# OpenwaterHealth/OpenLIFU-python

Measured on AMD Instinct MI355X. Metric: Mvoxel-elements/s pressure-field accumulate, higher is better.
Workload: dtype f32-acc/f16x2+e4m3-corr

## Files before the change

openlifu-python_amd/csrc/k_coset2.hip:

```cpp
#include <algorithm>
#include <cstdlib>
#include "k_types.hip.h"
#include "olx_ctx.h"
#include "olx_launch.h"

namespace olx {

constexpr int CP_TW = 14;
constexpr int CP_TROWS = 26, CP_ROW0 = 15;
constexpr int CP_PSZ = 364;
constexpr int CP_UW = 12;
constexpr int CP_SHARED = 4;
constexpr int CP_MT = 5;

#ifdef OLX_EXP_CUTRACE
static __device__ unsigned long long g_cutrace[16384][8][5];
#define OLX_CUTRACE(k, v) do { if (lane == 0 && blockIdx.y == 0 && blockIdx.x < 16384) g_cutrace[blockIdx.x][wave][k] = (v); } while (0)
#else
#define OLX_CUTRACE(k, v)
#endif

template <int MX, int MY, bool CLAMP, bool FP8, bool DIR = false, bool BOTH = true ,
          bool PONLY = false >
__global__ __launch_bounds__(COS_NW * 64, 4) void field_cosetp_k(
    const uint4* __restrict__ bfrag, float* __restrict__ pmag, float* __restrict__ inten,
    const int* __restrict__ targets ,
    const CosetBlock* __restrict__ blocks , const CosetParams P) {
    constexpr int NT = 2, THREADS = COS_NW * 64, PAIR = 2;
    static_assert(!(BOTH && PONLY), "one output or both");
    constexpr int TROWS = CP_TROWS, ROW0 = CP_ROW0, PSZ = CP_PSZ, MT = CP_MT;
    static_assert((PSZ / 2) % 2 == 0 && ((PSZ / 2) % 32 == 22 || (PSZ / 2) % 32 == 30), "16 planes on 16 distinct even 8-byte slots");
    constexpr int B_KS_U4 = 128;
    constexpr int B_BYTES = PAIR * 4 * NT * B_KS_U4 * 16;
    constexpr int T_WORDS = COS_ZB * PSZ;
    __shared__ __attribute__((aligned(16))) unsigned char smem[B_BYTES + T_WORDS * 4 + T_WORDS * 4 + 64];
    auto s_B = [&](int rec, int nt, int part) -> const uint4* { return reinterpret_cast<const uint4*>(smem) + ((size_t)(rec * NT + nt) * B_KS_U4 + part * 64); };
    unsigned* const s_hi = reinterpret_cast<unsigned*>(smem + B_BYTES);
    unsigned* const s_lo = s_hi + T_WORDS;
    const int tile = blockIdx.y;
    const int tid = threadIdx.x, lane = tid & 63, wave = __builtin_amdgcn_readfirstlane(tid >> 6);
    const int g = lane >> 4, p16 = lane & 15;
    OLX_CUTRACE(2, __builtin_readcyclecounter());
    OLX_CUTRACE(0, (unsigned long long)__builtin_amdgcn_s_getreg((31 << 11) | 4));
    OLX_CUTRACE(1, (unsigned long long)__builtin_amdgcn_s_getreg((31 << 11) | 20));
    const int item = blockIdx.x;
    {
    const CosetBlock BK = blocks[item];
    const int npos = BK.npos, KY = BK.KY, ky_magic = BK.ky_magic;
    if (npos <= 0) return;
    const int ibase = BK.ibase, jbase = BK.jbase;
    const int k0 = BK.k0;
    const int ntile = __builtin_amdgcn_readfirstlane((npos - wave + COS_NW - 1) / COS_NW);
    const int lane_off = p16 * PSZ - g * CP_TW;
    int toff[MT];
#pragma unroll
    for (int t = 0; t < MT; ++t) {
        const int pos = min(wave + COS_NW * t, npos - 1);
        const int kx = (pos * ky_magic) >> 16, ky = pos - kx * KY;
        toff[t] = (ky + ROW0) * CP_TW + (CP_UW - 8 - 2 * kx);
    }
    floatx4_t acc[MT][NT];
#pragma unroll
    for (int t = 0; t < MT; ++t)
#pragma unroll
        for (int nt = 0; nt < NT; ++nt) acc[t][nt] = floatx4_t{0.f, 0.f, 0.f, 0.f};
    const int nsbp = P.nsbp;
    const int n_sb = P.nsa * nsbp;
    bool reuse_ok = nsbp == PAIR;
#ifdef OLX_DEV_PINS
    reuse_ok = reuse_ok && P.cp_noreuse == 0;
#endif
    constexpr int CHUNK_U4 = PAIR * 4 * NT * B_KS_U4, PRE = CHUNK_U4 / THREADS;
    static_assert(CHUNK_U4 % THREADS == 0, "chunk must split evenly over the block");
    uint4 pre[PRE];
    const uint4* const bsrc = bfrag + (size_t)tile * n_sb * (4 * NT * B_KS_U4);
#pragma unroll
    for (int q = 0; q < PRE; ++q) {
        const int idx = tid + q * THREADS;
        pre[q] = idx < n_sb * 4 * NT * B_KS_U4 ? bsrc[idx] : make_uint4(0, 0, 0, 0);
    }
    OLX_STAMP(0);
    for (int sb0 = 0; sb0 < n_sb; sb0 += PAIR) {
        const int sa = sb0 / nsbp, sbb0 = sb0 - sa * nsbp;
        if (sb0 > 0) __syncthreads();
        const bool reuse = sb0 > 0 && reuse_ok;
        if (sb0 == 0) OLX_STAMP(1);
        if (sb0 == 2) OLX_STAMP(7);
        if constexpr (FP8) __builtin_amdgcn_s_setprio(1);
        if (k0 + wave * COS_P < P.nz) {
            int lane_o = lane;
            asm volatile("" : "+v"(lane_o));
            float dz2[COS_P];
#pragma unroll
            for (int z = 0; z < COS_P; ++z) {
                const float dz = (float)(k0 + wave * COS_P + z) * P.hz - P.flat_ez;
                dz2[z] = dz * dz;
            }
            auto entry = [&](const float r2, const float dz2v, const float dx, const float dy, const int o, const bool ok) __attribute__((always_inline)) {
                float d2 = r2 + dz2v;
                if (CLAMP) d2 = fmaxf(d2, P.dmin2);
                const float ri = __builtin_amdgcn_rsqf(d2);
                const float ph = d2 * ri;
                float rs = ri * P.g_scale;
                if constexpr (DIR) rs *= table_mod(dx, dy, ph, ri, P.dir_wx, P.dir_wy, P.absorb_l2);
                float gr = rs * __builtin_amdgcn_cosf(ph), gi = rs * __builtin_amdgcn_sinf(ph);
                asm volatile("" : "+v"(gr), "+v"(gi));
                half2_t hi;
                if constexpr (FP8) hi = __builtin_convertvector(float2_t{gr, gi}, half2_t);
                else hi = __builtin_bit_cast(half2_t, __builtin_amdgcn_cvt_pkrtz(gr, gi));
                float lr, li;
                const unsigned hw = __builtin_bit_cast(unsigned, hi);
                asm("v_fma_mix_f32 %0, %1, -1.0, %2 op_sel:[0,0,0] op_sel_hi:[1,0,0]" : "=v"(lr) : "v"(hw), "v"(gr));
                asm("v_fma_mix_f32 %0, %1, -1.0, %2 op_sel:[1,0,0] op_sel_hi:[1,0,0]" : "=v"(li) : "v"(hw), "v"(gi));
                unsigned lo_word;
                if constexpr (FP8) {
                    short2_t w;
                    w = __builtin_amdgcn_cvt_scalef32_pk_fp8_f32(w, lr, li, 1.0f / COS_F8_LO, false);
                    w = __builtin_amdgcn_cvt_scalef32_pk_fp8_f32(w, gr, gi, 1.0f / COS_F8_HI, true);
                    lo_word = __builtin_bit_cast(unsigned, w);
                } else {
                    lo_word = __builtin_bit_cast(unsigned, __builtin_amdgcn_cvt_pkrtz(lr, li));
                }
                if (ok && OLX_IN(o, T_WORDS, 0)) {
                    s_hi[o] = __builtin_bit_cast(unsigned, hi);
                    s_lo[o] = lo_word;
                }
            };
            auto fill = [&](auto reuse_c) __attribute__((always_inline)) {
                constexpr bool RU = decltype(reuse_c)::value != 0;
                constexpr int CW = RU ? CP_UW - CP_SHARED : CP_UW;
                constexpr int RPF = 64 / CW;
                constexpr int NRF = (TROWS - (RU ? COS_P : 1)) / RPF;
                static_assert(NRF * RPF == TROWS - (RU ? COS_P : 1) && (RU ? COS_P * COS_P : COS_P) <= RPF, "the tail rows fit one evaluation of the wave's planes");
                const int wl = lane_o / CW, ui = lane_o - CW * wl;
                const bool gen_lane = wl < RPF;
                const int Ulane = ibase + P.x_begin + P.ux0 + P.mx * (ui - 7);
                const int Wlane = jbase + P.uy0 + P.my * (wl - ROW0);
                const int tw_off = (wave * COS_P) * PSZ + wl * CP_TW + (CP_UW - 1 - ui);
                const float U = (float)(Ulane - 8 * P.mx * sa);
                const float dx = fmaf(U, P.hx_hi, fmaf(U, P.hx_lo, P.fx0));
                const float dx2 = dx * dx;
                const int Wsb = Wlane - 8 * P.my * sbb0;
#pragma unroll 2
                for (int r = 0; r < NRF; ++r) {
                    const float W = (float)(Wsb + RPF * P.my * r);
                    const float dy = fmaf(W, P.hy_hi, fmaf(W, P.hy_lo, P.fy0));
                    const float r2 = fmaf(dy, dy, dx2);
#pragma unroll
                    for (int z = 0; z < COS_P; ++z) entry(r2, dz2[z], dx, dy, z * PSZ + tw_off + RPF * r * CP_TW, gen_lane);
                }
                const bool last_row = KY + 14 >= TROWS - 1;
                if constexpr (RU) {
                    const int zt = wl >> 1, rowt = TROWS - COS_P + (wl & 1);
                    const float W = (float)(Wsb - P.my * wl + rowt * P.my);
                    const float dy = fmaf(W, P.hy_hi, fmaf(W, P.hy_lo, P.fy0));
                    float dzl = dz2[0];
#pragma unroll
                    for (int z = 1; z < COS_P; ++z) dzl = zt == z ? dz2[z] : dzl;
                    entry(fmaf(dy, dy, dx2), dzl, dx, dy, (wave * COS_P + zt) * PSZ + rowt * CP_TW + (CP_UW - 1 - ui), zt < COS_P && (last_row || rowt < TROWS - 1));
                } else if (last_row) {
                    const float W = (float)(Wsb - P.my * wl + (TROWS - 1) * P.my);
                    const float dy = fmaf(W, P.hy_hi, fmaf(W, P.hy_lo, P.fy0));
                    float dzl = dz2[0];
#pragma unroll
                    for (int z = 1; z < COS_P; ++z) dzl = wl == z ? dz2[z] : dzl;
                    entry(fmaf(dy, dy, dx2), dzl, dx, dy, (wave * COS_P + wl) * PSZ + (TROWS - 1) * CP_TW + (CP_UW - 1 - ui), wl < COS_P);
                }
            };
            if (reuse) {
                static_assert(COS_P * TROWS <= 64 && CP_UW - CP_SHARED == 8 && CP_TW % 2 == 0 && PSZ % 2 == 0, "one lane per (plane, row); aligned 8-byte moves");
                const int zm = lane_o >= TROWS ? 1 : 0;
                const int mo = (wave * COS_P + zm) * PSZ + (lane_o - zm * TROWS) * CP_TW;
                if (lane_o < COS_P * TROWS && OLX_IN(mo, T_WORDS - (CP_UW - 1), 3)) {
                    unsigned long long mv[4];
                    __builtin_memcpy(&mv[0], __builtin_assume_aligned(s_hi + mo + 8, 8), 8);
                    __builtin_memcpy(&mv[1], __builtin_assume_aligned(s_hi + mo + 10, 8), 8);
                    __builtin_memcpy(&mv[2], __builtin_assume_aligned(s_lo + mo + 8, 8), 8);
                    __builtin_memcpy(&mv[3], __builtin_assume_aligned(s_lo + mo + 10, 8), 8);
                    __builtin_memcpy(__builtin_assume_aligned(s_hi + mo, 8), &mv[0], 8);
                    __builtin_memcpy(__builtin_assume_aligned(s_hi + mo + 2, 8), &mv[1], 8);
                    __builtin_memcpy(__builtin_assume_aligned(s_lo + mo, 8), &mv[2], 8);
                    __builtin_memcpy(__builtin_assume_aligned(s_lo + mo + 2, 8), &mv[3], 8);
                }
                __builtin_amdgcn_fence(__ATOMIC_RELEASE, "wavefront");
                fill(IntC<1>{});
            } else {
                fill(IntC<0>{});
            }
        }
        if constexpr (FP8) __builtin_amdgcn_s_setprio(0);
#pragma unroll
        for (int q = 0; q < PRE; ++q) reinterpret_cast<uint4*>(smem)[tid + q * THREADS] = pre[q];
        if (sb0 == 0) OLX_STAMP(2);
        __syncthreads();
        if (sb0 == 0) OLX_STAMP(3);
        {
            const int nxt = (sb0 + PAIR) * 4 * NT * B_KS_U4, lim = n_sb * 4 * NT * B_KS_U4;
#pragma unroll
            for (int q = 0; q < PRE; ++q) {
                const int idx = nxt + tid + q * THREADS;
                if (idx < lim) pre[q] = bsrc[idx];
            }
        }
#pragma unroll
        for (int sl = 0; sl < PAIR; ++sl) {
            if (sbb0 + sl >= P.nsb) break;
            if constexpr (FP8) {
#pragma unroll
                for (int kb = 0; kb < 2; ++kb) {
                    Half8Bits bh[2][NT];
                    intx8_t b8[NT];
#pragma unroll
                    for (int nt = 0; nt < NT; ++nt) {
#pragma unroll
                        for (int ka = 0; ka < 2; ++ka) {
                            bh[ka][nt].u = s_B(sl * 4 + 2 * kb + ka, nt, 0)[lane];
                            const uint4 q = s_B(sl * 4 + 2 * kb + ka, nt, 1)[lane];
                            b8[nt][4 * ka + 0] = (int)q.x; b8[nt][4 * ka + 1] = (int)q.y; b8[nt][4 * ka + 2] = (int)q.z; b8[nt][4 * ka + 3] = (int)q.w;
                        }
                    }
#pragma unroll
                    for (int t = 0; t < MT; ++t) {
                        if (t >= ntile) continue;
                        Half8Bits ah[2];
                        intx8_t a8;
                        int lo_t = lane_off;
                        asm volatile("" : "+v"(lo_t));
                        const int ro = lo_t + toff[t];
#pragma unroll
                        for (int ka = 0; ka < 2; ++ka) {
                            const int kso = 4 * ka - (4 * kb + 8 * sl) * CP_TW;
                            if (!OLX_IN(ro + kso, T_WORDS - 3, 1)) continue;
                            const unsigned long long* ph2 = reinterpret_cast<const unsigned long long*>(s_hi + ro + kso);
                            const unsigned long long* pl2 = reinterpret_cast<const unsigned long long*>(s_lo + ro + kso);
                            const unsigned long long h0 = __hip_atomic_load(ph2, __ATOMIC_RELAXED, __HIP_MEMORY_SCOPE_WAVEFRONT);
                            const unsigned long long h1 = __hip_atomic_load(ph2 + 1, __ATOMIC_RELAXED, __HIP_MEMORY_SCOPE_WAVEFRONT);
                            const unsigned long long l0 = __hip_atomic_load(pl2, __ATOMIC_RELAXED, __HIP_MEMORY_SCOPE_WAVEFRONT);
                            const unsigned long long l1 = __hip_atomic_load(pl2 + 1, __ATOMIC_RELAXED, __HIP_MEMORY_SCOPE_WAVEFRONT);
                            ah[ka].w[0] = (unsigned)h0; ah[ka].w[1] = (unsigned)(h0 >> 32); ah[ka].w[2] = (unsigned)h1; ah[ka].w[3] = (unsigned)(h1 >> 32);
                            a8[4 * ka + 0] = (int)(unsigned)l0; a8[4 * ka + 1] = (int)(unsigned)(l0 >> 32);
                            a8[4 * ka + 2] = (int)(unsigned)l1; a8[4 * ka + 3] = (int)(unsigned)(l1 >> 32);
                        }
#pragma unroll
                        for (int nt = 0; nt < NT; ++nt) acc[t][nt] = __builtin_amdgcn_mfma_f32_16x16x32_f16(ah[0].h, bh[0][nt].h, acc[t][nt], 0, 0, 0);
#pragma unroll
                        for (int nt = 0; nt < NT; ++nt) acc[t][nt] = __builtin_amdgcn_mfma_f32_16x16x32_f16(ah[1].h, bh[1][nt].h, acc[t][nt], 0, 0, 0);
#pragma unroll
                        for (int nt = 0; nt < NT; ++nt)
                            acc[t][nt] = __builtin_amdgcn_mfma_scale_f32_16x16x128_f8f6f4(a8, b8[nt], acc[t][nt], 0, 0, 0, 128, 0, 127);
                    }
                }
            } else {
#pragma unroll
                for (int ks = 0; ks < 4; ++ks) {
                    const int ka = ks & 1, kb = ks >> 1;
                    Half8Bits bh[NT], bl[NT];
#pragma unroll
                    for (int nt = 0; nt < NT; ++nt) {
                        bh[nt].u = s_B(sl * 4 + ks, nt, 0)[lane];
                        bl[nt].u = s_B(sl * 4 + ks, nt, 1)[lane];
                    }
                    const int kso = 4 * ka - (4 * kb + 8 * sl) * CP_TW;
#pragma unroll
                    for (int t = 0; t < MT; ++t) {
                        if (t >= ntile) continue;
                        Half8Bits ah, al;
                        int lo_t = lane_off;
                        asm volatile("" : "+v"(lo_t));
                        const int ro = lo_t + toff[t];
                        if (!OLX_IN(ro + kso, T_WORDS - 3, 1)) continue;
                        const unsigned long long* ph2 = reinterpret_cast<const unsigned long long*>(s_hi + ro + kso);
                        const unsigned long long* pl2 = reinterpret_cast<const unsigned long long*>(s_lo + ro + kso);
                        const unsigned long long h0 = __hip_atomic_load(ph2, __ATOMIC_RELAXED, __HIP_MEMORY_SCOPE_WAVEFRONT);
                        const unsigned long long h1 = __hip_atomic_load(ph2 + 1, __ATOMIC_RELAXED, __HIP_MEMORY_SCOPE_WAVEFRONT);
                        const unsigned long long l0 = __hip_atomic_load(pl2, __ATOMIC_RELAXED, __HIP_MEMORY_SCOPE_WAVEFRONT);
                        const unsigned long long l1 = __hip_atomic_load(pl2 + 1, __ATOMIC_RELAXED, __HIP_MEMORY_SCOPE_WAVEFRONT);
                        ah.w[0] = (unsigned)h0; ah.w[1] = (unsigned)(h0 >> 32); ah.w[2] = (unsigned)h1; ah.w[3] = (unsigned)(h1 >> 32);
                        al.w[0] = (unsigned)l0; al.w[1] = (unsigned)(l0 >> 32); al.w[2] = (unsigned)l1; al.w[3] = (unsigned)(l1 >> 32);
#pragma unroll
                        for (int nt = 0; nt < NT; ++nt) acc[t][nt] = __builtin_amdgcn_mfma_f32_16x16x32_f16(ah.h, bh[nt].h, acc[t][nt], 0, 0, 0);
#pragma unroll
                        for (int nt = 0; nt < NT; ++nt) acc[t][nt] = __builtin_amdgcn_mfma_f32_16x16x32_f16(al.h, bh[nt].h, acc[t][nt], 0, 0, 0);
#pragma unroll
                        for (int nt = 0; nt < NT; ++nt) acc[t][nt] = __builtin_amdgcn_mfma_f32_16x16x32_f16(ah.h, bl[nt].h, acc[t][nt], 0, 0, 0);
                    }
                }
            }
        }
        if (sb0 == 0) OLX_STAMP(4);
    }
    OLX_STAMP(5);
    int lane_e = lane;
    asm volatile("" : "+v"(lane_e));
    const int c16 = lane_e >> 2;
    const int kz = k0 + 4 * (lane_e & 3);
    const int src_lane4 = (16 * (lane_e & 3) + (lane_e >> 2)) * 4;
    const float s_p = P.out_scale, s_i = P.out_scale * P.out_scale * P.inten_scale;
    const bool want_p = PONLY || (P.flags & 1u) != 0, want_i = !PONLY && (P.flags & 2u) != 0;
    constexpr int NOUT = PONLY ? 1 : NT;
#pragma unroll
    for (int t = 0; t < MT; ++t) {
        if (t >= ntile) continue;
        float o[NOUT][4];
#pragma unroll
        for (int r = 0; r < 4; r += 2) {
            const float2_t re = {acc[t][0][r], acc[t][0][r + 1]}, im = {acc[t][1][r], acc[t][1][r + 1]};
            const float2_t m = __builtin_elementwise_fma(re, re, im * im);
            o[0][r] = __builtin_amdgcn_sqrtf(m.x) * s_p;
            o[0][r + 1] = __builtin_amdgcn_sqrtf(m.y) * s_p;
            if constexpr (!PONLY) {
                const float2_t in = m * float2_t{s_i, s_i};
                o[1][r] = in.x;
                o[1][r + 1] = in.y;
            }
        }
#pragma unroll
        for (int nt = 0; nt < NOUT; ++nt) {
            floatx4_t v;
            v[0] = __builtin_bit_cast(float, __builtin_amdgcn_ds_bpermute(src_lane4, __builtin_bit_cast(int, o[nt][0])));
            v[1] = __builtin_bit_cast(float, __builtin_amdgcn_ds_bpermute(src_lane4, __builtin_bit_cast(int, o[nt][1])));
            v[2] = __builtin_bit_cast(float, __builtin_amdgcn_ds_bpermute(src_lane4, __builtin_bit_cast(int, o[nt][2])));
            v[3] = __builtin_bit_cast(float, __builtin_amdgcn_ds_bpermute(src_lane4, __builtin_bit_cast(int, o[nt][3])));
            acc[t][nt] = v;
        }
    }
    if (kz < P.nz) {
    const int4 tq = *reinterpret_cast<const int4*>(targets + ((size_t)tile * (MFMA_COLS * MFMA_MAX_NT) + c16) * 4);
    const int xm = P.nx - 1, ym = P.ny - 1;
    const int sxz = P.ny * P.nz;
    auto readout = [&](auto full_c) {
        constexpr bool FULL4 = decltype(full_c)::value != 0;
#pragma unroll
        for (int q = 0; q < 4; ++q) {
            const int code = q == 0 ? tq.x : q == 1 ? tq.y : q == 2 ? tq.z : tq.w;
            if (code < 0) continue;
            const unsigned m = (unsigned)code & 3u;
            const bool fx = (MX == 2) && (m & 1u), fy = (MY == 2) && ((MX == 2) ? (m >> 1) : (m & 1u));
            unsigned fxm = fx ? 0xFFFFFFFFu : 0u, fym = fy ? 0xFFFFFFFFu : 0u;
            asm volatile("" : "+v"(fxm), "+v"(fym));
            const long long fb = (long long)(code >> 2) * P.vox + kz;
            float* const base_p = pmag + fb;
            float* const base_i = inten + fb;
#pragma unroll
            for (int t = 0; t < MT; ++t) {
                if (t >= ntile) continue;
                const int pos = wave + COS_NW * t;
                const int kx = (pos * ky_magic) >> 16, ky = pos - kx * KY;
                const int i = ibase + 2 * P.mx * kx, j = jbase + P.my * ky;
                const unsigned o00 = (unsigned)(i * sxz + j * P.nz);
                const unsigned DX = (unsigned)((xm - 2 * i) * sxz), DY = (unsigned)((ym - 2 * j) * P.nz);
                const unsigned off = o00 + (fxm & DX) + (fym & DY);
                if (!OLX_IN(fb + off + (FULL4 ? 3 : 0), (long long)P.n_foci * P.vox, 2)) continue;
                if constexpr (FULL4) {
                    if (BOTH || PONLY || want_p) *reinterpret_cast<floatx4u_t*>(base_p + off) = floatx4u_t{acc[t][0][0], acc[t][0][1], acc[t][0][2], acc[t][0][3]};
                    if (!PONLY && (BOTH || want_i)) *reinterpret_cast<floatx4u_t*>(base_i + off) = floatx4u_t{acc[t][1][0], acc[t][1][1], acc[t][1][2], acc[t][1][3]};
                } else {
#pragma unroll
                    for (int e = 0; e < 4; ++e)
                        if (kz + e < P.nz) {
                            if (BOTH || PONLY || want_p) base_p[off + e] = acc[t][0][e];
                            if (!PONLY && (BOTH || want_i)) base_i[off + e] = acc[t][1][e];
                        }
                }
            }
        }
    };
    if (k0 + COS_ZB <= P.nz) readout(IntC<1>{}); else readout(IntC<0>{});
    }
    OLX_STAMP(6);
#ifdef OLX_EXP_CUTRACE
    OLX_CUTRACE(3, __builtin_readcyclecounter());
    asm volatile("s_waitcnt vmcnt(0)" ::: "memory");
    OLX_CUTRACE(4, __builtin_readcyclecounter());
#endif
    }
}

}

using namespace olx;
OLX_BOUNDS_READER(cosetp)

#ifdef OLX_EXP_CUTRACE
extern "C" int olx_exp_read_cutrace_cosetp(unsigned long long* out) {
    return (int)hipMemcpyFromSymbol(out, HIP_SYMBOL(olx::g_cutrace), sizeof(unsigned long long) * 16384 * 8 * 5);
}
#endif
#ifdef OLX_EXP_STAMPS
extern "C" int olx_exp_read_stamps_cosetp(unsigned long long* out) {
    return (int)hipMemcpyFromSymbol(out, HIP_SYMBOL(olx::g_stamps), sizeof(unsigned long long) * 4096 * 8);
}
#endif

template <int MX, int MY>
static void launch_cosetp(olx_ctx* c, const LatticePart& q, float* pm) {
    CosetParams Q = c->cp;
#ifdef OLX_DEBUG_BOUNDS
    if (getenv("OLX_DEBUG_BOUNDS_SELFTEST")) Q.n_foci -= 1;
#endif
    float* inten_exp = c->d_inten;
    const bool clamp = c->clamp || c->lat.clamp;
    dim3 grid(q.n_blocks, c->mp.n_tiles), blk(COS_NW * 64);
    const bool both = (Q.flags & 3u) == 3u, ponly = (Q.flags & 3u) == 1u;
#define OLX_CP(CL, F8, DR) do { if (both) hipLaunchKernelGGL((field_cosetp_k<MX, MY, CL, F8, DR, true, false>), grid, blk, 0, c->stream, q.bfrag, pm, inten_exp, c->d_targets, q.blocks, Q); \
                                else if (ponly) hipLaunchKernelGGL((field_cosetp_k<MX, MY, CL, F8, DR, false, true>), grid, blk, 0, c->stream, q.bfrag, pm, inten_exp, c->d_targets, q.blocks, Q); \
                                else hipLaunchKernelGGL((field_cosetp_k<MX, MY, CL, F8, DR, false, false>), grid, blk, 0, c->stream, q.bfrag, pm, inten_exp, c->d_targets, q.blocks, Q); } while (0)
    if (c->dir_lattice) {
        if (clamp) OLX_CP(true, false, true); else OLX_CP(false, false, true);
    } else if (q.fp8) {
        if (clamp) OLX_CP(true, true, false); else OLX_CP(false, true, false);
    } else {
        if (clamp) OLX_CP(true, false, false); else OLX_CP(false, false, false);
    }
#undef OLX_CP
}

void olx_launch_cosetp(olx_ctx* c, const LatticePart& q, float* pm) {
    if (c->mx == 2 && c->my == 2) launch_cosetp<2, 2>(c, q, pm);
    else if (c->mx == 2) launch_cosetp<2, 1>(c, q, pm);
    else if (c->my == 2) launch_cosetp<1, 2>(c, q, pm);
    else launch_cosetp<1, 1>(c, q, pm);
}
```

openlifu-python_amd/csrc/olx.hip:

```cpp
#include "olx_ctx.h"

#include <dlfcn.h>
#include <unistd.h>

#include <algorithm>
#include <climits>
#include <cmath>
#include <cstring>
#include <thread>

#include "k_small.hip.h"
#include "olx_launch.h"
#include "olx_plan.h"
#include "k_toep.hip.h"

OLX_BOUNDS_READER(small)

template <class T> static int upload_if_changed(olx_ctx* c, DevBuf<T>& d, std::vector<T>& held, const std::vector<T>& v) {
    if (d.capacity() < v.size() || !d) held.clear();
    { int rc = d.reserve(c, v.size()); if (rc) return rc; }
    if (held.size() == v.size() && (v.empty() || !memcmp(held.data(), v.data(), sizeof(T) * v.size()))) return OLX_OK;
    HIPCHK(c, hipMemcpyAsync(d, v.data(), sizeof(T) * v.size(), hipMemcpyHostToDevice, c->stream));
    HIPCHK(c, hipStreamSynchronize(c->stream));
    held = v;
// ... 384 lines not shown
    c->bc_planes = (int)zp.size();
    c->bc_valid = true;
    return OLX_OK;
}

int olx_bf_solve_compensated(olx_ctx* c, const double* foci_m, int n_foci, const double* M, double cs, int apod_kind,
                             double p0, double p1, int mode, int spreading, int use_delay_medium, double* delays_out, double* apod_out) {
    if (!c) return OLX_EINVAL;
    if (!c->ba_set) return fail(c, OLX_ESTATE, "olx_bf_solve_compensated: call olx_bf_set_attenuation first");
    if (use_delay_medium && !c->bm_set) return fail(c, OLX_ESTATE, "olx_bf_solve_compensated: call olx_bf_set_medium first (use_delay_medium)");
    if (c->n_el <= 0) return fail(c, OLX_ESTATE, "olx_bf_solve_compensated: call olx_set_elements first");
    if (!foci_m || n_foci <= 0) return fail(c, OLX_EINVAL, "olx_bf_solve_compensated: no foci");
    if (mode != OLX_COMP_EQUALIZE && mode != OLX_COMP_MATCHED) return fail(c, OLX_EINVAL, "olx_bf_solve_compensated: unknown mode %d", mode);
    if (use_delay_medium) {
        const BfMedParams &a = c->bm, &b = c->ba;
        if (cs != a.c) return fail(c, OLX_EINVAL, "olx_bf_solve_compensated: c (%.17g) must be the c_ref of olx_bf_set_medium (%.17g)", cs, a.c);
        if (a.nx != b.nx || a.ny != b.ny || a.nz != b.nz || a.ox != b.ox || a.oy != b.oy || a.oz != b.oz || a.hx != b.hx || a.hy != b.hy || a.hz != b.hz)
            return fail(c, OLX_EINVAL, "olx_bf_solve_compensated: the media of olx_bf_set_medium and olx_bf_set_attenuation must share one grid");
    }
    for (size_t q = 0; q < 3 * (size_t)n_foci; ++q)
        if (!std::isfinite(foci_m[q])) return fail(c, OLX_EINVAL, "olx_bf_solve_compensated: focus positions must be finite");
    for (int q = 0; M && q < 16; ++q)
        if (!std::isfinite(M[q])) return fail(c, OLX_EINVAL, "olx_bf_solve_compensated: transform must be finite");
    int rc = olx_bf_solve(c, foci_m, n_foci, M, cs, apod_kind, p0, p1, nullptr, nullptr);
    if (rc) return rc;
    const size_t fn = (size_t)n_foci * c->n_el;
    rc = c->d_ba_h.reserve(c, fn);
    if (!rc && use_delay_medium && !c->bc_valid) rc = build_joint_walk(c);
    if (rc) { c->n_foci = 0; return rc; }
    olx_launch_bfapod(c, n_foci, mode, spreading != 0, use_delay_medium != 0);
    HIPCHK(c, hipGetLastError());
    if (use_delay_medium) HIPCHK(c, hipMemcpyAsync(c->h_delays.data(), c->d_delays, sizeof(double) * fn, hipMemcpyDeviceToHost, c->stream));
    HIPCHK(c, hipMemcpyAsync(c->h_apod.data(), c->d_apod, sizeof(double) * fn, hipMemcpyDeviceToHost, c->stream));
    HIPCHK(c, hipStreamSynchronize(c->stream));
    if (delays_out) memcpy(delays_out, c->h_delays.data(), sizeof(double) * fn);
    if (apod_out) memcpy(apod_out, c->h_apod.data(), sizeof(double) * fn);
    c->steer_version++;
    if (use_delay_medium) c->h_foci.clear();
    else if (!c->h_foci.empty()) c->foci_version = c->steer_version;
    c->bf_valid = false;
    return OLX_OK;
}

int olx_set_steering(olx_ctx* c, const double* delays_s, const double* apod, int n_foci) {
    if (!c) return OLX_EINVAL;
    if (c->n_el <= 0) return fail(c, OLX_ESTATE, "olx_set_steering: call olx_set_elements first");
    if (!delays_s || !apod || n_foci <= 0) return fail(c, OLX_EINVAL, "olx_set_steering: null pointer or n_foci <= 0");
    HIPCHK(c, hipSetDevice(c->device));
    const size_t fn = (size_t)n_foci * c->n_el;
    int rc = c->d_delays.reserve(c, fn);
    if (!rc) rc = c->d_apod.reserve(c, fn);
    if (rc) return rc;
    HIPCHK(c, hipMemcpyAsync(c->d_delays, delays_s, sizeof(double) * fn, hipMemcpyHostToDevice, c->stream));
    HIPCHK(c, hipMemcpyAsync(c->d_apod, apod, sizeof(double) * fn, hipMemcpyHostToDevice, c->stream));
    HIPCHK(c, hipStreamSynchronize(c->stream));
    c->h_delays.assign(delays_s, delays_s + fn); c->h_apod.assign(apod, apod + fn);
    c->h_foci.clear();
    c->bf_valid = false;
    c->n_foci = n_foci;
    c->steer_version++;
    return OLX_OK;
}

int olx_bf_quantize(olx_ctx* c, double bf_clk_hz, int width_bits, uint16_t* ticks_out, uint8_t* apod_off_out,
                    double* max_apod_out, int32_t* n_overflow_out) {
    if (!c) return OLX_EINVAL;
    if (c->n_foci <= 0) return fail(c, OLX_ESTATE, "olx_bf_quantize: no steering table (olx_bf_solve / olx_set_steering)");
    if (!(bf_clk_hz > 0) || width_bits < 1 || width_bits > 16) return fail(c, OLX_EINVAL, "olx_bf_quantize: bad clock or width");
    HIPCHK(c, hipSetDevice(c->device));
    const int F = c->n_foci, n = c->n_el;
    const size_t fn = (size_t)F * n;
    DevScratch scratch;
    const size_t off_o = sizeof(double) * F, off_t = off_o + sizeof(int) * (size_t)((F + 1) & ~1), off_a = off_t + sizeof(unsigned short) * fn;
    HIPCHK(c, hipMalloc(&scratch.p, off_a + fn));
    double* d_m = scratch.at<double>(0);
    int* d_o = scratch.at<int>(off_o);
    unsigned short* d_t = scratch.at<unsigned short>(off_t);
    unsigned char* d_a = scratch.at<unsigned char>(off_a);
    hipLaunchKernelGGL(bf_quantize_k, dim3(F), dim3(BF_THREADS), 0, c->stream, c->d_delays, c->d_apod, n, bf_clk_hz,
                       (1u << width_bits) - 1u, d_t, d_a, d_m, d_o);
    int rc = OLX_OK;
    if (hipGetLastError() != hipSuccess) rc = fail(c, OLX_EHIP, "olx_bf_quantize: launch failed");
    if (!rc && ticks_out && hipMemcpyAsync(ticks_out, d_t, sizeof(unsigned short) * fn, hipMemcpyDeviceToHost, c->stream) != hipSuccess) rc = OLX_EHIP;
    if (!rc && apod_off_out && hipMemcpyAsync(apod_off_out, d_a, fn, hipMemcpyDeviceToHost, c->stream) != hipSuccess) rc = OLX_EHIP;
    if (!rc && max_apod_out && hipMemcpyAsync(max_apod_out, d_m, sizeof(double) * F, hipMemcpyDeviceToHost, c->stream) != hipSuccess) rc = OLX_EHIP;
    if (!rc && n_overflow_out && hipMemcpyAsync(n_overflow_out, d_o, sizeof(int) * F, hipMemcpyDeviceToHost, c->stream) != hipSuccess) rc = OLX_EHIP;
    if (hipStreamSynchronize(c->stream) != hipSuccess && !rc) rc = OLX_EHIP;
    if (rc == OLX_EHIP) return fail(c, OLX_EHIP, "olx_bf_quantize: HIP error");
    return rc;
}

using olxplan::build_slot_map;
using olxplan::coset_tiles16;
static void detect_lattice(olx_ctx* c, const double lo[3], const double hi[3], double dmin) {
    olxplan::detect_lattice(c->lat, c->flat, c->n_el, c->h_pos.data(), c->grid.spacing, lo, hi, dmin);
}
static bool infer_foci(const olx_ctx* c, std::vector<double>& foci) {
    const int n = c->n_el, F = c->plan_foci;
    if (c->h_delays.size() != (size_t)F * n) return false;
    return olxplan::infer_foci(c->flat, n, F, c->h_pos.data(), c->h_delays.data(), c->c,
                               c->grid.origin[2] + 0.5 * (c->grid.n[2] - 1) * c->grid.spacing[2], foci);
}

static int configure_variant_impl(olx_ctx* c);
static int configure_variant(olx_ctx* c) {
    c->configured_version = ~0ull;
    const int rc = configure_variant_impl(c);
    if (rc == OLX_OK) c->configured_version = c->steer_version;
    return rc;
}
static int configure_variant_impl(olx_ctx* c) {
    const int n = c->n_el, F = c->plan_foci;
    const char* const fv_env = getenv("OLX_FIELD_VARIANT");
    auto steering_symmetric = [&](const std::vector<int>& perm) {
        if (c->h_delays.size() != (size_t)F * n || c->h_apod.size() != (size_t)F * n) return false;
        for (int f = 0; f < F; ++f)
            for (int e = 0; e < n; ++e) {
                const size_t a = (size_t)f * n + e, b = (size_t)f * n + perm[e];
                if (std::fabs(c->h_delays[a] - c->h_delays[b]) * c->freq > 1e-9) return false;
                if (std::fabs(c->h_apod[a] * c->h_area[e] - c->h_apod[b] * c->h_area[perm[e]]) >
                    1e-12 * std::fabs(c->h_apod[a] * c->h_area[e])) return false;
            }
        return true;
    };
    if (c->hetero) {
        c->mx = c->my = c->dx = c->dy = c->nt = 1; c->use_mfma = false; c->use_lattice = false;
        c->nf = 1;
        while (c->nf * 2 <= F && c->nf < 8) c->nf *= 2;
        { int rc = c->d_tab.reserve(c, (size_t)((F + c->nf - 1) / c->nf) * n * (HET_TAB_HEAD + 2 * c->nf)); if (rc) return rc; }
        c->hp.n_foci = F;
        char hb[160];
        if (c->marched)
            snprintf(hb, sizeof hb, "field_hmarch_k<nf%d,%s%s> (%d non-trivial planes, marched ray sums, %d launches)", c->nf,
                     c->clamp ? "clamp" : "noclamp", c->march_one ? ",one-sum" : "", c->hp.n_planes, 2 * c->hp.n_planes + 1);
        else if (c->hp.n_layers > 0)
            snprintf(hb, sizeof hb, "field_hetero_k<4,nf%d,%s,layers> (%d non-trivial planes in %d layers of <= %d)", c->nf,
                     c->clamp ? "clamp" : "noclamp", c->hp.n_planes, c->hp.n_layers, c->planes_per_layer);
        else
            snprintf(hb, sizeof hb, "field_hetero_k<4,nf%d,%s> (%d non-trivial planes)", c->nf, c->clamp ? "clamp" : "noclamp", c->hp.n_planes);
        c->variant = hb;
        return OLX_OK;
    }
    c->dx = (c->mx == 2 && !steering_symmetric(c->h_px)) ? 2 : 1;
    c->dy = (c->my == 2 && !steering_symmetric(c->h_py)) ? 2 : 1;
    const int nm = c->dx * c->dy;
    c->nf = 1;
    if (c->allow_shared) while (c->nf * 2 <= F && c->nf * 2 * nm <= 8) c->nf *= 2;
    char nmbuf[384];
    auto tile_fill = [](int width, int m) { const int blk = 4 * m; return (double)width / (double)(((width + blk - 1) / blk) * blk); };
    const bool lat_ok = c->allow_shared && c->lat.ok && (c->force_kind == 0 || c->force_kind == 4) &&
                        tile_fill(c->fp.nx - (c->mx == 2 ? c->fp.nx / 2 : 0), c->lat.mx) >= 0.5 &&
                        tile_fill(c->fp.ny - (c->my == 2 ? c->fp.ny / 2 : 0), c->lat.my) >= 0.5;
    if (c->modifier() && !(lat_ok && c->dir_lattice)) {
        c->allow_shared = false; c->dir_lattice = false;
        c->mx = c->my = c->dx = c->dy = c->nf = 1;
    }
    c->use_mfma = c->allow_shared && c->force_kind != 2 && (c->force_kind == 3 || nm * c->nf >= 2 || lat_ok) && (!c->modifier() || lat_ok);
    c->use_lattice = c->use_mfma && lat_ok;
    c->fp8corr = false;
    c->nt = 1;
    if (c->use_mfma) {
        const double rev = c->freq / c->c, lambda = c->c / c->freq;
        const int n_img = c->mx * c->my;
        constexpr int MAXC = MFMA_COLS * MFMA_MAX_NT;
        const std::vector<int> perm = olxplan::mirror_perms(n, n_img, c->mx == 2, c->my == 2, c->h_px.data(), c->h_py.data(), 4);
        olxplan::Steering SV;
        SV.n = n; SV.F = F; SV.n_img = n_img; SV.perm = perm.data(); SV.delays = c->h_delays.data(); SV.apod = c->h_apod.data(); SV.area = c->h_area.data(); SV.freq = c->freq;
        typedef olxplan::Col Col;
        auto pack = [&](int maxc) { return olxplan::pack_columns(SV, maxc); };
        auto coset_fill = [&](int nt) {
            const int wx = c->fp.nx - (c->mx == 2 ? c->fp.nx / 2 : 0), wy = c->fp.ny - (c->my == 2 ? c->fp.ny / 2 : 0);
            const long long t16 = coset_tiles16(wx, wy, c->lat.mx, c->lat.my, nt);
            return t16 > 0 ? (double)COS_P * wx * wy / (16.0 * (double)t16) : 0.0;
        };
        auto fp8_eligible = [&]() -> int {
            if ((c->flags & (OLX_FIELD_FP16_CORRECTION | OLX_OUT_COMPLEX)) || c->modifier() || !c->lat.ok) return -1;
            bool ok = c->h_foci.size() == 3 * (size_t)F && c->foci_version == c->steer_version;
            if (!ok && infer_foci(c, c->h_foci)) {
                c->foci_version = c->steer_version;
                ok = true;
            }
            if (!ok) return -1;
            return olxplan::fp8_first_plane(n, c->h_pos.data(), c->h_area.data(), c->h_apod.data(), F, c->h_foci.data(), c->grid.origin, c->grid.spacing,
                                            c->grid.n, c->slab.x_begin, c->slab.x_count, c->lat, c->nf_s2);
        };
        const char* f8env = getenv("OLX_FP8_CORRECTION");
        int fp8_cut = (lat_ok && !(f8env && !strcmp(f8env, "0"))) ? fp8_eligible() : -1;
#ifdef OLX_DEV_PINS
        if (f8env && strcmp(f8env, "0") != 0) fp8_cut = (lat_ok && !c->modifier()) ? 0 : -1;
#endif
        if (fp8_cut > 0 && !olxplan::fp8_split_pays(c->slab.x_count, c->grid.n[1], c->grid.n[2], F, fp8_cut)) fp8_cut = -1;
        const bool fp8_want = fp8_cut >= 0;
        c->fp8_kcut = fp8_want ? fp8_cut : 0;
        olxplan::Tiles tiles = pack(MAXC);
        int total_cols = 0;
        {
            const bool wide = tiles.size() == 1 && (int)tiles[0].size() > MFMA_COLS * 2;
            if ((tiles.size() > 1 || (wide && fp8_want)) && c->use_lattice && !(c->flags & OLX_OUT_COMPLEX) && !fv_env && coset_fill(2) >= 0.6) {
                tiles = pack(MFMA_COLS * 2);
            }
        }
        c->nt = 1;
        for (auto& t : tiles) { total_cols += (int)t.size(); while (c->nt * MFMA_COLS < (int)t.size()) c->nt *= 2; }
        if (c->use_lattice && c->nt >= 4 && c->force_kind != 4 && ((c->flags & OLX_OUT_COMPLEX) || coset_fill(c->nt) < 0.6)) c->use_lattice = false;
        c->use_coset = false; c->use_toep = false; c->use_cosetp = false;
        if (c->use_lattice) {
            const char* fv = fv_env;
            if (c->modifier() && fv && strcmp(fv, "lattice") && strcmp(fv, "lattice2d")) fv = nullptr;
            c->use_coset = !(c->flags & OLX_OUT_COMPLEX) && !(fv && !strcmp(fv, "lattice2d"));
            if (coset_fill(c->nt) > 0 && coset_fill(c->nt) < 0.6 && !(fv && !strcmp(fv, "lattice"))) c->use_coset = false;
            const int want = (c->use_coset && c->nt <= 2) ? ((c->lat.nsb + 1) & ~1) : c->lat.nsb;
            if (want != c->lat.nsbp) build_slot_map(c->lat, want);
            c->use_toep = c->use_coset && tiles.size() == 1 && total_cols == 1 && !(fv && !strcmp(fv, "lattice"));
            c->use_cosetp = c->use_coset && !c->use_toep && c->nt == 2 && !(fv && !strcmp(fv, "lattice"));
            if (c->use_cosetp)
                olxplan::balance_store_targets(tiles, c->nt * MFMA_COLS);
        }
        const int n_pad = c->use_lattice ? c->lat.n_pad : (n + 15) / 16 * 16;
        const int ntiles = (int)tiles.size();
        const size_t n_col = (size_t)ntiles * MAXC;
        std::vector<int> colinfo(n_col * 6, -1);
        for (int t = 0; t < ntiles; ++t)
            for (size_t o = 0; o < tiles[t].size(); ++o) {
                colinfo[((size_t)t * MAXC + o) * 2] = tiles[t][o].f;
                colinfo[((size_t)t * MAXC + o) * 2 + 1] = tiles[t][o].m;
                for (int q = 0; q < 4; ++q) colinfo[n_col * 2 + ((size_t)t * MAXC + o) * 4 + q] = tiles[t][o].tgt[q];
            }
        { int rc = upload_if_changed(c, c->d_perm, c->up_perm, perm); if (rc) return rc; }
        { int rc = upload_if_changed(c, c->d_colinfo, c->up_colinfo, colinfo); if (rc) return rc; }
        c->d_targets = c->d_colinfo + n_col * 2;
        c->bfrag_half = (size_t)ntiles * (n_pad / 16) * 128 * c->nt;
        {
            int rc = c->d_coords.reserve(c, 2 * (size_t)n_pad);
            if (!rc) rc = c->d_bfrag.reserve(c, 2 * c->bfrag_half);
            if (rc) return rc;
        }
        const double dmin_m = 0.5 * std::min({c->grid.spacing[0], c->grid.spacing[1], c->grid.spacing[2]});
        const bool lat_clamp = c->use_lattice && (c->clamp || c->lat.clamp);
        const double min_dist = !c->use_lattice ? c->min_dist : (lat_clamp ? dmin_m : std::sqrt(c->lat.min_d2));
        if (c->use_lattice) {
            int rc = upload_if_changed(c, c->d_slot, c->up_slot, c->lat.slot_elem);
            if (rc) return rc;
        }
        const double dmin_w = std::max(min_dist * rev, 1e-6);
        const double sg = std::exp2(std::floor(std::log2(16384.0 * dmin_w)));
        double wmax = 0;
        for (size_t q = 0; q < (size_t)F * n; ++q) wmax = std::max(wmax, std::fabs(c->h_apod[q] * c->h_area[q % n]));
        wmax *= c->p0_pa / lambda * rev;
        const double sw = wmax > 0 ? std::exp2(std::floor(std::log2(16384.0 / wmax))) : 1.0;
        const FieldParams& P = c->fp;
        MfmaParams& M = c->mp;
        M.nx = P.nx; M.ny = P.ny; M.nz = P.nz; M.n_el_pad = n_pad; M.x_begin = P.x_begin; M.n_tiles = ntiles;
        M.hx = P.hx; M.hy = P.hy; M.hz = P.hz; M.dmin2 = P.dmin2; M.flat_ez = P.flat_ez; M.flat_kz = P.flat_kz; M.flat_fz = P.flat_fz;
        M.g_scale = (float)sg; M.out_scale = (float)(1.0 / (sg * sw)); M.inten_scale = P.inten_scale;
        M.vox = P.vox; M.flags = P.flags;
        c->mfma_wscale = c->p0_pa / lambda * rev * sw;
        if (c->use_lattice) {
            const olx_ctx::Lattice& A = c->lat;
            LatParams& L = c->lp;
            c->lat_mt = 4;
            L.nx = P.nx; L.ny = P.ny; L.nz = P.nz;
            L.x_lo = c->mx == 2 ? P.nx / 2 : 0; L.y_lo = c->my == 2 ? P.ny / 2 : 0; L.x_begin = P.x_begin;
            L.mx = A.mx; L.my = A.my;
            L.tiles_x = ((P.nx - L.x_lo + 4 * A.mx - 1) / (4 * A.mx)) * 2 * A.mx;
            L.tiles_y = ((P.ny - L.y_lo + 4 * A.my - 1) / (4 * A.my)) * A.my;
            L.kgroups = (P.nz + 2 * c->lat_mt - 1) / (2 * c->lat_mt);
            L.nsa = A.nsa; L.nsb = A.nsb; L.nsbp = A.nsbp;
            const double offx = c->grid.origin[0] - A.x0, offy = c->grid.origin[1] - A.y0;
            L.ux0 = (int)std::llround(offx / c->grid.spacing[0]); L.uy0 = (int)std::llround(offy / c->grid.spacing[1]);
            L.fx0 = (float)((offx - L.ux0 * c->grid.spacing[0]) * rev); L.fy0 = (float)((offy - L.uy0 * c->grid.spacing[1]) * rev);
            const double hxw = c->grid.spacing[0] * rev, hyw = c->grid.spacing[1] * rev;
            L.hx_hi = (float)hxw; L.hx_lo = (float)(hxw - (double)L.hx_hi);
            L.hy_hi = (float)hyw; L.hy_lo = (float)(hyw - (double)L.hy_hi);
            L.hz = P.hz; L.dmin2 = P.dmin2; L.flat_ez = P.flat_ez;
            L.g_scale = M.g_scale; L.out_scale = M.out_scale; L.inten_scale = P.inten_scale;
            L.vox = P.vox; L.flags = P.flags;
            const long long tiles16 = coset_tiles16(P.nx - L.x_lo, P.ny - L.y_lo, A.mx, A.my, c->nt);
            c->fp8corr = fp8_want && c->use_coset && cos_fp8(c->nt) && !c->modifier();
            if (c->use_coset) {
                CosetParams& Q = c->cp;
                Q.nx = L.nx; Q.ny = L.ny; Q.nz = L.nz; Q.x_lo = L.x_lo; Q.y_lo = L.y_lo; Q.x_begin = L.x_begin; Q.mx = L.mx; Q.my = L.my;
                const int zb = COS_ZB;
                Q.xs = c->use_toep ? 1 : 2;
                olxplan::ToepPlan tp{};
                c->toep_nm = 1;
                int kyw = COS_KYW;
                if (c->use_toep) {
                    int saw_pin = 0, nm_pin = 0;
#ifdef OLX_DEV_PINS
                    if (const char* e = getenv("OLX_EXP_TOEP_SAW")) { const int v = atoi(e); if (v >= 8 && v <= 24) saw_pin = v; }
                    if (const char* e = getenv("OLX_EXP_TOEP_NM")) nm_pin = atoi(e) == 3 ? 3 : 1;
#endif
                    tp = olxplan::toep_plan(A.ax, Q.mx, Q.my, Q.xs, Q.nx - Q.x_lo, Q.ny - Q.y_lo, Q.nz, c->dir_lattice, saw_pin, nm_pin);
                    c->toep_nm = tp.nm; kyw = tp.kyw;
                }
                const int kxw = c->use_toep ? 8 * c->toep_nm : cos_kxw(c->nt);
                olxplan::coset_partition(Q, kxw, zb, kyw);
                Q.nsa = L.nsa; Q.nsb = L.nsb; Q.nsbp = L.nsbp; Q.ux0 = L.ux0; Q.uy0 = L.uy0; Q.fx0 = L.fx0; Q.fy0 = L.fy0;
                Q.hx_hi = L.hx_hi; Q.hx_lo = L.hx_lo; Q.hy_hi = L.hy_hi; Q.hy_lo = L.hy_lo; Q.hz = L.hz;
                Q.dmin2 = L.dmin2; Q.flat_ez = L.flat_ez; Q.g_scale = L.g_scale; Q.out_scale = L.out_scale; Q.inten_scale = L.inten_scale;
                Q.vox = L.vox; Q.flags = L.flags; Q.n_foci = F;
#ifdef OLX_DEV_PINS
                { const char* e = getenv("OLX_EXP_CP_NOREUSE"); Q.cp_noreuse = (e && atoi(e) != 0) ? 1 : 0; }
#endif
                Q.dir_wx = (c->dir_lattice && c->directivity) ? (float)(0.5 * c->h_size[0] / lambda) : 0.f;
                Q.dir_wy = (c->dir_lattice && c->directivity) ? (float)(0.5 * c->h_size[1] / lambda) : 0.f;
                Q.absorb_l2 = c->dir_lattice ? (float)(c->absorb_np_m * lambda * 1.4426950408889634) : 0.f;
                {
                    const std::vector<int> jobs = olxplan::build_store_jobs(tiles, MFMA_MAX_NT, MFMA_COLS, COS_JOBS, (P.flags & OLX_OUT_PMAG) != 0, (P.flags & OLX_OUT_INTENSITY) != 0);
                    int rc = upload_if_changed(c, c->d_jobs, c->up_jobs, jobs);
                    if (rc) return rc;
                }
                {
                    auto pick_grp = [&](int kblocks) {
                        const unsigned long long nb = (unsigned long long)Q.xs * Q.mx * Q.my * Q.nsx * Q.nsy * kblocks;
                        for (int g2 = std::min(kblocks, 32); g2 >= 2; --g2) if (kblocks % g2 == 0 && nb % (8ull * g2) == 0) return (unsigned)g2;
                        return 1u;
                    };
                    const int kcut = c->fp8corr ? c->fp8_kcut : 0;
                    const int kb_near = kcut / zb, kb_far = Q.kblocks - kb_near;
                    unsigned kgrp = pick_grp(kb_far), kgrp_near = kb_near > 0 ? pick_grp(kb_near) : 0u;
#ifdef OLX_DEV_PINS
                    if (const char* e = getenv("OLX_EXP_KGRP")) { kgrp = (unsigned)std::max(1, atoi(e)); if (kb_near > 0) kgrp_near = kgrp; }
#endif
                    const int rec_key[16] = {Q.nx, Q.ny, Q.nz, Q.x_lo, Q.y_lo, Q.mx, Q.my, Q.nsx, Q.nsy, Q.kblocks, zb, (int)kgrp, c->use_cosetp ? 40 : 0, Q.xs, kcut, (int)kgrp_near};
                    std::vector<CosetBlock> blk;
                    if (!c->up_blocks.empty() && memcmp(c->up_blocks_key, rec_key, sizeof rec_key) == 0) blk = c->up_blocks;
                    else {
                        std::string why;
                        CosetParams Qf = Q; Qf.kblocks = kb_far;
                        if (!olxplan::build_coset_blocks(Qf, zb, kgrp, c->use_cosetp ? 40 : 0, blk, why))
                            return fail(c, OLX_ESTATE, "kernel 2g: %s", why.c_str());
                        for (CosetBlock& b : blk) b.k0 += kcut;
                        if (kb_near > 0) {
                            std::vector<CosetBlock> near;
                            CosetParams Qn = Q; Qn.kblocks = kb_near;
                            if (!olxplan::build_coset_blocks(Qn, zb, kgrp_near, c->use_cosetp ? 40 : 0, near, why))
                                return fail(c, OLX_ESTATE, "kernel 2g: %s", why.c_str());
                            blk.insert(blk.end(), near.begin(), near.end());
                        }
                    }
                    const unsigned nblk = (unsigned)blk.size();
                    c->cp_nfar = nblk - (unsigned)((unsigned long long)Q.xs * Q.mx * Q.my * Q.nsx * Q.nsy * kb_near);
                    { int rc = upload_if_changed(c, c->d_cpblocks, c->up_blocks, blk); if (rc) return rc; }
                    memcpy(c->up_blocks_key, rec_key, sizeof rec_key);
                    c->cp_nblocks = nblk;
                }
                const double far_frac = c->fp8corr ? (double)std::max(0, P.nz - c->fp8_kcut) / (double)P.nz : 0.0;
                const double corr_units = 3.0 - far_frac;
                const std::string f8tag = !c->fp8corr ? "" : (c->fp8_kcut > 0 ? ",fp8corr from plane " + std::to_string(c->fp8_kcut) : ",fp8corr");
                const long long n_dense = (long long)((double)(P.nx - L.x_lo) * (P.ny - L.y_lo) * P.nz * (double)n * total_cols * 4.0 / 8192.0 * corr_units);
                if (c->use_toep) {
                    c->toep_saw = tp.saw;
                    c->toep_nsa = tp.nsa;
                    if (c->toep_nsa > 16) return fail(c, OLX_ESTATE, "kernel 2f: more than 16 super-block columns");
                    c->toep_ksmask = tp.ks_mask;
                    const int ksteps_total = tp.ksteps_total, e4_units = tp.e4_units;
                    for (int q = 0; q < 4; ++q) c->toep_targets[q] = tiles[0][0].tgt[q];
                    { int rc = c->d_cell.reserve(c, A.cell.size()); if (rc) return rc; }
                    HIPCHK(c, hipMemcpy(c->d_cell, A.cell.data(), sizeof(int) * A.cell.size(), hipMemcpyHostToDevice));
                    c->afrag_half = (size_t)ntiles * c->toep_nsa * 8 * A.nsb * 4 * 64;
                    { int rc = c->d_afrag.reserve(c, 2 * c->afrag_half); if (rc) return rc; }
                    long long n_mfma = 0;
                    const int wx = P.nx - L.x_lo, wy = P.ny - L.y_lo;
                    const double units_e4m3 = c->toep_nm == 2 ? 3.0 : (double)ksteps_total + (double)e4_units;
                    const double per_row = far_frac * units_e4m3 + (1.0 - far_frac) * 3.0 * ksteps_total;
                    for (int rx = 0; rx < Q.xs * A.mx; ++rx)
                        for (int ry = 0; ry < A.my; ++ry) {
                            const int kxa = rx < wx ? (wx - 1 - rx) / (Q.xs * A.mx) + 1 : 0, kya = ry < wy ? (wy - 1 - ry) / A.my + 1 : 0;
                            for (int sx = 0; sx < Q.nsx; ++sx)
                                for (int sy = 0; sy < Q.nsy; ++sy) {
                                    const int KX = (sx + 1) * kxa / Q.nsx - sx * kxa / Q.nsx, KY = (sy + 1) * kya / Q.nsy - sy * kya / Q.nsy;
                                    if (KX > 0 && KY > 0) n_mfma += (long long)((double)KY * per_row * (c->toep_nm > 1 ? 8 * c->toep_nm : 8) * A.nsb * Q.kblocks);
                                }
                        }
                    snprintf(nmbuf, sizeof nmbuf, "field_toep%s_k<mx%d,my%d,flat,%s%s> %d columns for %d foci x %d images in %d tile(s); "
                             "%dx%d lattice, pitch %dx%d voxels, %lld MFMA/launch (%lld dense), %d row tile(s) x %d y positions per block", "", c->mx, c->my, lat_clamp ? "clamp" : "noclamp", f8tag.c_str(),
                             total_cols, F, n_img, ntiles, A.ax, A.ay, A.mx, A.my, n_mfma, n_dense, c->toep_nm, kyw);
                } else {
                long long n_mfma = (long long)((double)tiles16 * ((P.nz + COS_P - 1) / COS_P) * A.nsa * A.nsb * 4 * c->nt * corr_units * ntiles);
                if (c->use_cosetp) {
                    long long npos_all = 0;
                    const int wx = P.nx - L.x_lo, wy = P.ny - L.y_lo;
                    for (int rx = 0; rx < 2 * A.mx; ++rx)
                        for (int ry = 0; ry < A.my; ++ry)
                            npos_all += (long long)(rx < wx ? (wx - 1 - rx) / (2 * A.mx) + 1 : 0) * (ry < wy ? (wy - 1 - ry) / A.my + 1 : 0);
                    n_mfma = (long long)((double)npos_all * Q.kblocks * A.nsa * A.nsb * 4 * c->nt * corr_units * ntiles);
                }
#ifdef OLX_DEV_PINS
                const char* const noreuse_tag = (c->use_cosetp && Q.cp_noreuse) ? ",noreuse" : "";
#else
                const char* const noreuse_tag = "";
#endif
                snprintf(nmbuf, sizeof nmbuf, "field_coset%s_k<nt%d,mx%d,my%d,flat,%s%s%s> %d columns for %d foci x %d images in %d tile(s); "
                         "%dx%d lattice, pitch %dx%d voxels, %lld MFMA/launch (%lld dense)", c->use_cosetp ? "p" : "", c->nt, c->mx, c->my, lat_clamp ? "clamp" : "noclamp",
                         f8tag.c_str(), noreuse_tag, total_cols, F, n_img, ntiles, A.ax, A.ay, A.mx, A.my, n_mfma, n_dense);
                }
            } else {
                const long long n_mfma = (long long)L.tiles_x * L.tiles_y * L.kgroups * A.nsa * A.nsb * 4 * c->lat_mt * c->nt * 3 * ntiles;
                snprintf(nmbuf, sizeof nmbuf, "field_lattice_k<mt%d,nt%d,mx%d,my%d,flat,%s> %d columns for %d foci x %d images in %d tile(s); "
                         "%dx%d lattice, pitch %dx%d voxels, %lld MFMA/launch", c->lat_mt, c->nt, c->mx, c->my, lat_clamp ? "clamp" : "noclamp",
                         total_cols, F, n_img, ntiles, A.ax, A.ay, A.mx, A.my, n_mfma);
            }
        } else {
            snprintf(nmbuf, sizeof nmbuf, "field_mfma_k<mt%d,nt%d,mx%d,my%d,%s,%s> %d columns for %d foci x %d images in %d tile(s)",
                     P.nz >= 48 ? 4 : 1, c->nt, c->mx, c->my, c->flat ? "flat" : "general", c->clamp ? "clamp" : (c->near ? "near" : "noclamp"), total_cols, F,
                     n_img, ntiles);
        }
    } else if (c->mx * c->my * c->nf == 1) {
        if (c->modifier()) snprintf(nmbuf, sizeof nmbuf, "field_accum_dir_k<4,%s> (%s%s%s)", c->clamp ? "clamp" : "noclamp", c->directivity ? "piston directivity" : "",
                                    (c->directivity && c->absorb_np_m > 0) ? ", " : "", c->absorb_np_m > 0 ? "uniform absorption" : "");
        else snprintf(nmbuf, sizeof nmbuf, "field_accum_k<4,%s,%s>", c->flat ? "flat" : "general", c->clamp ? "clamp" : (c->near ? "near" : "noclamp"));
    } else {
        const std::vector<int> perm = olxplan::mirror_perms(n, nm, c->dx == 2, c->dy == 2, c->h_px.data(), c->h_py.data(), nm);
        int rc = upload_if_changed(c, c->d_perm, c->up_perm, perm);
        if (!rc) rc = c->d_tab.reserve(c, (size_t)((F + c->nf - 1) / c->nf) * n * (SH_HEAD + 2 * nm * c->nf));
        if (rc) return rc;
        snprintf(nmbuf, sizeof nmbuf, "field_shared_k<4,mx%d,my%d,dx%d,dy%d,nf%d,%s,%s>", c->mx, c->my, c->dx, c->dy, c->nf,
                 c->flat ? "flat" : "general", c->clamp ? "clamp" : (c->near ? "near" : "noclamp"));
    }
    if (c->modifier() && c->use_mfma && !(c->use_lattice && c->use_coset)) {
        c->dir_lattice = false; c->allow_shared = false;
        return configure_variant_impl(c);
    }
    if (c->directivity && c->use_mfma) strncat(nmbuf, " +piston directivity in the tables", sizeof nmbuf - strlen(nmbuf) - 1);
    if (c->absorb_np_m > 0 && c->use_mfma) strncat(nmbuf, " +uniform absorption in the tables", sizeof nmbuf - strlen(nmbuf) - 1);
    c->variant = nmbuf;
    return OLX_OK;
}

static LatticePart lattice_part(const olx_ctx* c, bool below) {
    if (below) return {c->d_bfrag + c->bfrag_half, c->d_afrag + c->afrag_half, c->d_cpblocks + c->cp_nfar, c->cp_nblocks - c->cp_nfar, false};
    const bool split = c->fp8corr && c->cp_nfar < c->cp_nblocks;
    return {c->d_bfrag, c->d_afrag, c->d_cpblocks, split ? c->cp_nfar : c->cp_nblocks, c->fp8corr};
}

static int pack_if_needed(olx_ctx* c) {
    if (c->packed_version == c->steer_version) return OLX_OK;
    if (c->configured_version != c->steer_version) { int rc = configure_variant(c); if (rc) return rc; }
    const double lambda = c->c / c->freq;
    if (c->hetero) {
        olx_pack_hetero(c);
    } else if (c->use_mfma) {
        const double ox = c->mx == 2 ? c->grid.origin[0] + 0.5 * (c->grid.n[0] - 1) * c->grid.spacing[0] : c->grid.origin[0];
        const double oy = c->my == 2 ? c->grid.origin[1] + 0.5 * (c->grid.n[1] - 1) * c->grid.spacing[1] : c->grid.origin[1];
        dim3 g(c->mp.n_el_pad / 16, c->mp.n_tiles, c->nt);
        hipLaunchKernelGGL(mfma_pack_k, g, dim3(64), 0, c->stream, c->d_pos, c->d_area, c->n_el, c->mp.n_el_pad, c->d_delays,
                           c->d_apod, c->d_perm, ox, oy, c->grid.origin[2], c->freq, c->mfma_wscale, c->freq / c->c,
                           c->plan_foci, c->d_colinfo, c->use_lattice ? c->d_slot : nullptr,
                           (c->use_lattice && c->use_coset && c->fp8corr) ? 1 : 0, (c->use_lattice && c->use_cosetp) ? 1 : 0,
                           c->near ? (c->mx == 2 ? 0.5 : 1.0) * c->grid.spacing[0] : 0.0, (c->my == 2 ? 0.5 : 1.0) * c->grid.spacing[1], c->grid.spacing[2], c->d_coords, c->d_bfrag);
        if (c->use_lattice && c->use_toep) olx_pack_toep(c, lattice_part(c, false));
        if (c->use_lattice && c->use_coset && c->fp8corr && c->cp_nfar < c->cp_nblocks) {
            hipLaunchKernelGGL(mfma_pack_k, g, dim3(64), 0, c->stream, c->d_pos, c->d_area, c->n_el, c->mp.n_el_pad, c->d_delays,
                               c->d_apod, c->d_perm, ox, oy, c->grid.origin[2], c->freq, c->mfma_wscale, c->freq / c->c,
                               c->plan_foci, c->d_colinfo, c->d_slot, 0, c->use_cosetp ? 1 : 0, 1.0, 1.0, 1.0, c->d_coords, c->d_bfrag + c->bfrag_half);
            if (c->use_toep) olx_pack_toep(c, lattice_part(c, true));
        }
    } else if (c->mx * c->my * c->nf == 1) {
        dim3 g((c->n_el + 127) / 128, c->plan_foci);
        c->tab_split = c->near || c->modifier();
        hipLaunchKernelGGL(steer_pack_k, g, dim3(128), 0, c->stream, c->d_pos, c->d_area, c->n_el, c->d_delays,
                           c->d_apod, c->grid.origin[0], c->grid.origin[1], c->grid.origin[2], c->freq,
                           c->p0_pa / lambda, c->freq / c->c, nullptr, nullptr, c->tab_split ? c->grid.spacing[0] : 0.0, c->grid.spacing[1], c->grid.spacing[2], c->d_tab);
        if (c->directivity) {
            const int n = c->n_el;
            std::vector<float> t2((size_t)n * 8);
            for (int e = 0; e < n; ++e) {
                const double* x = &c->h_xaxis[3 * (size_t)e]; const double* nr = &c->h_nrm[3 * (size_t)e];
                const double y[3] = {nr[1] * x[2] - nr[2] * x[1], nr[2] * x[0] - nr[0] * x[2], nr[0] * x[1] - nr[1] * x[0]};
                float* t = &t2[(size_t)e * 8];
                t[0] = (float)x[0]; t[1] = (float)x[1]; t[2] = (float)x[2]; t[3] = (float)(0.5 * c->h_size[2 * (size_t)e] / lambda);
                t[4] = (float)y[0]; t[5] = (float)y[1]; t[6] = (float)y[2]; t[7] = (float)(0.5 * c->h_size[2 * (size_t)e + 1] / lambda);
            }
            { int rc = c->d_tab2.reserve(c, t2.size()); if (rc) return rc; }
            HIPCHK(c, hipMemcpyAsync(c->d_tab2, t2.data(), sizeof(float) * t2.size(), hipMemcpyHostToDevice, c->stream));
            HIPCHK(c, hipStreamSynchronize(c->stream));
        }
    } else {
        const double ox = c->mx == 2 ? c->grid.origin[0] + 0.5 * (c->grid.n[0] - 1) * c->grid.spacing[0] : c->grid.origin[0];
        const double oy = c->my == 2 ? c->grid.origin[1] + 0.5 * (c->grid.n[1] - 1) * c->grid.spacing[1] : c->grid.origin[1];
        const int tiles = (c->plan_foci + c->nf - 1) / c->nf;
        dim3 g((c->n_el + 127) / 128, tiles);
        hipLaunchKernelGGL(steer_pack_shared_k, g, dim3(128), 0, c->stream, c->d_pos, c->d_area, c->n_el, c->d_delays,
                           c->d_apod, c->d_perm, ox, oy, c->grid.origin[2], c->freq, c->p0_pa / lambda, c->freq / c->c,
                           c->plan_foci, c->nf, c->dx * c->dy, c->near ? (c->mx == 2 ? 0.5 : 1.0) * c->grid.spacing[0] : 0.0, (c->my == 2 ? 0.5 : 1.0) * c->grid.spacing[1], c->grid.spacing[2], c->d_tab);
    }
    HIPCHK(c, hipGetLastError());
    c->packed_version = c->steer_version;
    return OLX_OK;
}

}

static int plan_pulse(olx_ctx* c, const olx_grid* g, const olx_slab* slab, int n_foci, double freq, double cs, double rho, double p0_pa,
                      unsigned flags) {
    if (flags & ~(OLX_OUT_PMAG | OLX_OUT_INTENSITY | OLX_OUT_PMAX | OLX_OUT_PII | OLX_FIELD_FP8_CORRECTION | OLX_FIELD_FP16_CORRECTION))
        return fail(c, OLX_EINVAL, "olx_field_plan: a pulsed plan (olx_field_pulse) takes OLX_OUT_PMAG / OLX_OUT_INTENSITY / OLX_OUT_PMAX / OLX_OUT_PII only "
                    "(no complex output, no OLX_FIELD_DIRECTIVITY), flags 0x%x", flags);
    if (slab && !(slab->x_begin == 0 && slab->x_count == g->n[0]))
        return fail(c, OLX_EINVAL, "olx_field_plan: a pulsed plan (olx_field_pulse) covers the whole grid: no slab");
    if (c->comm_active()) return fail(c, OLX_ESTATE, "olx_field_plan: a pulsed plan (olx_field_pulse) has no multi-GPU path: destroy the communicator first");
    const long long vox = (long long)g->n[0] * g->n[1] * g->n[2];
    if (vox > (1ll << 31) * 4) return fail(c, OLX_EINVAL, "olx_field_plan: grid too large for a pulsed plan");
    HIPCHK(c, hipSetDevice(c->device));
    HIPCHK(c, hipStreamSynchronize(c->stream));
    const size_t total = (size_t)vox * n_foci;
    c->grid = *g; c->slab = olx_slab{0, g->n[0]}; c->plan_foci = n_foci; c->hetero = false; c->marched = false;
    c->agg_local = -1; c->agg_total = 0;
    c->freq = freq; c->c = cs; c->rho = rho; c->p0_pa = p0_pa; c->flags = flags; c->plan_absorb = c->absorb_np_m;
    c->directivity = false; c->nbuf = 1; c->cur = 0;
    const size_t fn = (size_t)n_foci * c->n_el;
    pii_regrid(c, vox);
    c->derive_i = false; c->inten_live = false;
    int rc = reserve_outputs(c, total, 1, (flags & OLX_OUT_INTENSITY) != 0, false, false);
    if (!rc && (flags & OLX_OUT_PMAX)) rc = c->d_pmax.reserve(c, total);
    if (!rc && (flags & OLX_OUT_PII)) rc = c->d_pii.reserve(c, total);
    if (!rc) rc = c->d_ptab.reserve(c, fn);
    if (!rc) rc = c->d_pw.reserve(c, fn);
    if (rc) return rc;
    FieldParams& F = c->fp;
    F.nx = g->n[0]; F.ny = g->n[1]; F.nz = g->n[2]; F.n_el = c->n_el; F.x_begin = 0; F.vox = vox;
    F.flags = (flags & 3u) | OLX_OUT_PMAG; F.inten_scale = (float)(1e-4 / (2.0 * rho * cs));
    PulseParams& P = c->pulse;
    const double dt = c->pulse_dt;
    c->pulse_plan_dt = dt;
    P.n_el = c->n_el; P.n_foci = n_foci; P.n_t = c->pulse_nt; P.ny = g->n[1]; P.nz = g->n[2];
    P.ox = g->origin[0]; P.oy = g->origin[1]; P.oz = g->origin[2];
    P.hx = g->spacing[0]; P.hy = g->spacing[1]; P.hz = g->spacing[2];
    P.dmin = 0.5 * std::min({g->spacing[0], g->spacing[1], g->spacing[2]});
    P.inv_cdt = 1.0 / (cs * dt);
    P.tdt = c->pulse_cycles / (freq * dt);
    P.f0dt = freq * dt;
    P.dmin_f = (float)P.dmin; P.inv_cdt_f = (float)P.inv_cdt;
    P.absorb = (float)c->absorb_np_m;
    P.rot_c = (float)std::cos(2.0 * M_PI * P.f0dt); P.rot_s = (float)std::sin(2.0 * M_PI * P.f0dt);
    P.inten_scale = F.inten_scale;
    P.pii_scale = (float)(1e-4 * dt / (rho * cs));
    P.vox = vox;
    c->pulsed = true; c->pmax_live = false; c->agg_pmax_valid = false; c->pii_live = false;
    char nm[128];
    snprintf(nm, sizeof nm, "field_pulse_k (pulsed: %d samples, %.4g samples per burst)", c->pulse_nt, P.tdt);
    c->variant = nm;
    c->packed_version = ~0ull;
    c->planned = true; c->uploaded = false;
    return OLX_OK;
}

extern "C" {

int olx_field_plan(olx_ctx* c, const olx_grid* g, const olx_slab* slab, int n_foci, double freq, double cs,
                   double rho, double p0_pa, unsigned flags) {
    if (!c) return OLX_EINVAL;
    if (c->n_el <= 0) return fail(c, OLX_ESTATE, "olx_field_plan: call olx_set_elements first");
    if (c->n_foci <= 0) return fail(c, OLX_ESTATE, "olx_field_plan: no steering table (olx_bf_solve / olx_set_steering)");
    if (!g) return fail(c, OLX_EINVAL, "olx_field_plan: null grid");
    if (n_foci != c->n_foci) return fail(c, OLX_EINVAL, "olx_field_plan: n_foci %d != steering table foci %d", n_foci, c->n_foci);
    for (int a = 0; a < 3; ++a)
        if (g->n[a] < 1 || !(g->spacing[a] > 0)) return fail(c, OLX_EINVAL, "olx_field_plan: bad grid axis %d", a);
    if (!(freq > 0) || !(cs > 0) || !(rho > 0)) return fail(c, OLX_EINVAL, "olx_field_plan: freq, c, rho must be > 0");
    if (!(flags & (OLX_OUT_PMAG | OLX_OUT_INTENSITY | OLX_OUT_COMPLEX))) return fail(c, OLX_EINVAL, "olx_field_plan: no outputs selected");
    if (c->pulse_nt > 0) return plan_pulse(c, g, slab, n_foci, freq, cs, rho, p0_pa, flags);
    if (flags & OLX_OUT_PMAX) return fail(c, OLX_EINVAL, "olx_field_plan: OLX_OUT_PMAX needs a pulsed plan (olx_field_pulse)");
    if (flags & OLX_OUT_PII) return fail(c, OLX_EINVAL, "olx_field_plan: OLX_OUT_PII needs a pulsed plan (olx_field_pulse)");
    if (flags & ~(OLX_OUT_PMAG | OLX_OUT_INTENSITY | OLX_OUT_COMPLEX | OLX_FIELD_FP8_CORRECTION | OLX_FIELD_FP16_CORRECTION | OLX_FIELD_DIRECTIVITY)) return fail(c, OLX_EINVAL, "olx_field_plan: unknown flag bits 0x%x", flags);
    if ((flags & OLX_FIELD_DIRECTIVITY) && c->h_xaxis.size() != 3 * (size_t)c->n_el)
        return fail(c, OLX_ESTATE, "olx_field_plan: OLX_FIELD_DIRECTIVITY needs olx_set_element_apertures");
    olx_slab s{0, g->n[0]};
    if (slab) s = *slab;
    if (s.x_begin < 0 || s.x_count < 1 || s.x_begin + s.x_count > g->n[0]) return fail(c, OLX_EINVAL, "olx_field_plan: slab outside grid");
    HIPCHK(c, hipSetDevice(c->device));
    {
        std::string env;
        for (const char* name : {"OLX_FIELD_VARIANT", "OLX_FP8_CORRECTION", "OLX_EXP_TOEP_SAW", "OLX_EXP_TOEP_NM", "OLX_EXP_KGRP", "OLX_INTENSITY_STORED", "OLX_EXP_CP_NOREUSE"}) { const char* e = getenv(name); env += e ? e : ""; env += '|'; }
        const bool same = c->planned && !c->uploaded && !c->hetero && !c->pulsed && memcmp(&c->grid, g, sizeof *g) == 0 && c->slab.x_begin == s.x_begin &&
                          c->slab.x_count == s.x_count && c->plan_foci == n_foci && c->freq == freq && c->c == cs && c->rho == rho &&
                          c->p0_pa == p0_pa && c->flags == flags && c->plan_absorb == c->absorb_np_m && c->nbuf == (c->comm_active() ? olx_ctx::NBUF : 1) && c->plan_env == env;
        c->plan_env = env;
        if (same) {
            c->agg_local = -1; c->agg_total = 0;
            if (c->packed_version != c->steer_version) return configure_variant(c);
            return OLX_OK;
        }
    }
    HIPCHK(c, hipStreamSynchronize(c->stream));
    c->grid = *g; c->slab = s; c->plan_foci = n_foci; c->hetero = false;
    c->pulsed = false; c->pmax_live = false; c->agg_pmax_valid = false; c->pii_live = false;
    c->agg_local = -1; c->agg_total = 0;
    c->freq = freq; c->c = cs; c->rho = rho; c->p0_pa = p0_pa; c->flags = flags; c->plan_absorb = c->absorb_np_m;
    const long long vox = (long long)s.x_count * g->n[1] * g->n[2];
    pii_regrid(c, vox);
    const size_t total = (size_t)vox * n_foci;
    c->nbuf = c->comm_active() ? olx_ctx::NBUF : 1;
    { const char* pin = getenv("OLX_INTENSITY_STORED"); c->derive_i = (flags & OLX_OUT_INTENSITY) && !(pin && *pin && strcmp(pin, "0") != 0); }
    c->inten_live = false;
    { int rc = reserve_outputs(c, total, c->nbuf, (flags & OLX_OUT_INTENSITY) && !c->derive_i, (flags & OLX_OUT_COMPLEX) != 0, true); if (rc) return rc; }
    if (c->derive_i) c->d_inten.release();
    { int rc = c->d_tab.reserve(c, (size_t)n_foci * c->n_el * TAB_STRIDE); if (rc) return rc; }
    FieldParams& P = c->fp;
    P.nx = s.x_count; P.ny = g->n[1]; P.nz = g->n[2]; P.n_el = c->n_el;
    P.x_begin = s.x_begin;
    const double rev = freq / cs;
    P.hx = (float)(g->spacing[0] * rev); P.hy = (float)(g->spacing[1] * rev); P.hz = (float)(g->spacing[2] * rev);
    const double dmin = 0.5 * std::min({g->spacing[0], g->spacing[1], g->spacing[2]});
    P.dmin2 = (float)(dmin * dmin * rev * rev);
    P.inten_scale = (float)(1e-4 / (2.0 * rho * cs));
    P.vox = vox; P.flags = ((flags & 7u) | OLX_OUT_PMAG) & ~(c->derive_i ? (unsigned)OLX_OUT_INTENSITY : 0u);
    c->directivity = (flags & OLX_FIELD_DIRECTIVITY) != 0;
    const int n = c->n_el;
    const double* hz = c->h_pos.data() + 2 * (size_t)n;
    c->flat = true;
    for (int e = 1; e < n; ++e) if (hz[e] != hz[0]) { c->flat = false; break; }
    P.flat_ez = (float)((hz[0] - g->origin[2]) * rev);
    { const double kz = std::rint((hz[0] - g->origin[2]) / g->spacing[2]); P.flat_kz = (float)kz; P.flat_fz = (float)(((hz[0] - g->origin[2]) - kz * g->spacing[2]) * rev); }
    double lo[3], hi[3];
    for (int a = 0; a < 3; ++a) {
        const int b = (a == 0) ? s.x_begin : 0;
        const int cnt = (a == 0) ? s.x_count : g->n[a];
        lo[a] = g->origin[a] + b * g->spacing[a];
        hi[a] = g->origin[a] + (b + cnt - 1) * g->spacing[a];
    }
    c->clamp = false;
    const double guard = 2.0 * dmin;
    double min_d2 = 1e300;
    for (int e = 0; e < n; ++e) {
        double d2 = 0;
        for (int a = 0; a < 3; ++a) {
            const double p = c->h_pos[(size_t)a * n + e];
            const double d = p < lo[a] ? lo[a] - p : (p > hi[a] ? p - hi[a] : 0.0);
            d2 += d * d;
        }
        min_d2 = std::min(min_d2, d2);
        if (d2 < guard * guard) c->clamp = true;
    }
    c->min_dist = c->clamp ? dmin : std::sqrt(min_d2);
    c->near = c->clamp || c->min_dist < 0.25 * cs / freq;
    detect_lattice(c, lo, hi, dmin);
    c->nf_s2.clear();
    auto mirror_perm = [&](int axis, std::vector<int>& perm) -> bool {
        const double ctr = g->origin[axis] + 0.5 * (g->n[axis] - 1) * g->spacing[axis];
        const double tol = 1e-12;
        perm.assign(n, -1);
        std::vector<char> used(n, 0);
        for (int e = 0; e < n; ++e) {
            const double want = 2.0 * ctr - c->h_pos[(size_t)axis * n + e];
            int hit = -1;
            for (int o = 0; o < n && hit < 0; ++o) {
                if (used[o] || std::fabs(c->h_pos[(size_t)axis * n + o] - want) > tol) continue;
                bool same = true;
                for (int a = 0; a < 3; ++a)
                    if (a != axis && std::fabs(c->h_pos[(size_t)a * n + o] - c->h_pos[(size_t)a * n + e]) > tol) same = false;
                if (same) hit = o;
            }
            if (hit < 0) return false;
            used[hit] = 1; perm[e] = hit;
        }
        return true;
    };
    const bool whole_x = (s.x_begin == 0 && s.x_count == g->n[0]);
    const char* force = getenv("OLX_FIELD_VARIANT");
    c->force_kind = !force ? 0 : !strcmp(force, "general") ? 1 : !strcmp(force, "shared") ? 2 : !strcmp(force, "mfma") ? 3 : (!strcmp(force, "lattice") || !strcmp(force, "lattice2d")) ? 4 : 0;
    c->dir_lattice = false;
    P.absorb_l2 = (float)(c->absorb_np_m * (cs / freq) * 1.4426950408889634);
    if (c->modifier() && !(flags & OLX_OUT_COMPLEX) && c->flat) {
        bool ok = !c->directivity || (c->h_xaxis.size() == 3 * (size_t)n && c->h_size.size() == 2 * (size_t)n);
        for (int e = 0; c->directivity && ok && e < n; ++e) {
            const double* xa = &c->h_xaxis[3 * (size_t)e]; const double* nr = &c->h_nrm[3 * (size_t)e];
            if (std::fabs(std::fabs(xa[0]) - 1.0) > 1e-12 || std::fabs(xa[1]) > 1e-12 || std::fabs(xa[2]) > 1e-12) ok = false;
            if (std::fabs(std::fabs(nr[2]) - 1.0) > 1e-12) ok = false;
            if (c->h_size[2 * (size_t)e] != c->h_size[0] || c->h_size[2 * (size_t)e + 1] != c->h_size[1]) ok = false;
        }
        c->dir_lattice = ok;
    }
    c->allow_shared = c->force_kind != 1 && c->force_kind != 5 && (!c->modifier() || c->dir_lattice);
    c->mx = (c->allow_shared && whole_x && g->n[0] >= 2 && n <= 8192 && mirror_perm(0, c->h_px)) ? 2 : 1;
    c->my = (c->allow_shared && g->n[1] >= 2 && n <= 8192 && mirror_perm(1, c->h_py)) ? 2 : 1;
    {
        int rc = c->d_tab.reserve(c, ((size_t)n_foci * 12 + 24) * n);
        if (c->d_perm.capacity() < (size_t)4 * n) c->up_perm.clear();
        if (!rc) rc = c->d_perm.reserve(c, (size_t)4 * n);
        if (rc) return rc;
    }
    SharedParams& S = c->sp;
    S.nx = P.nx; S.ny = P.ny; S.nz = P.nz; S.n_el = n; S.x_begin = s.x_begin; S.n_foci = n_foci;
    S.hx = P.hx; S.hy = P.hy; S.hz = P.hz; S.dmin2 = P.dmin2;
    S.inten_scale = P.inten_scale; S.flat_ez = P.flat_ez; S.flat_kz = P.flat_kz; S.flat_fz = P.flat_fz; S.vox = P.vox; S.flags = P.flags;
    c->dx = c->mx; c->dy = c->my; c->nf = 1;
    char nm[96] = "(steering-dependent)";
    c->variant = nm;
    c->packed_version = ~0ull;
    c->planned = true; c->uploaded = false;
    c->cur = 0;
    return configure_variant(c);
}

}

extern "C" {

int olx_field_launch(olx_ctx* c) {
    if (!c) return OLX_EINVAL;
    if (!c->planned) return fail(c, OLX_ESTATE, "olx_field_launch: call olx_field_plan first");
    if (c->uploaded) return fail(c, OLX_ESTATE, "olx_field_launch: resident volumes were uploaded, not planned");
    if (c->n_foci != c->plan_foci) return fail(c, OLX_ESTATE, "olx_field_launch: steering table changed shape since plan");
    HIPCHK(c, hipSetDevice(c->device));
    if (c->pulsed) {
        if (c->flags & OLX_OUT_PMAX) c->pmax_live = false;
        c->agg_pmax_valid = false; c->pii_live = false; c->pii_w_valid = false; c->pii_max_valid = false;
        const bool prof = c->prof_on && (size_t)(2 * c->prof_n + 1) < c->prof_ev.size();
        if (prof) HIPCHK(c, hipEventRecord(c->prof_ev[2 * c->prof_n], c->stream));
        olx_launch_pulse(c, c->d_pmag[0]);
        HIPCHK(c, hipGetLastError());
        if (prof) { HIPCHK(c, hipEventRecord(c->prof_ev[2 * c->prof_n + 1], c->stream)); c->prof_n++; }
        c->pmax_live = (c->flags & OLX_OUT_PMAX) != 0;
        c->pii_live = (c->flags & OLX_OUT_PII) != 0; c->pii_foci = c->plan_foci;
        c->cur = 0;
        return OLX_OK;
    }
    int rc = pack_if_needed(c);
    if (rc) return rc;
    const int b = (c->nbuf == 2) ? (c->cur ^ 1) : 0;
    if (c->gather_pending[b]) {
        if (c->p2p) { rc = olx_p2p_before_overwrite(c, b); if (rc) { c->gather_pending[b] = false; return rc; } }
        else HIPCHK(c, hipStreamWaitEvent(c->stream, c->ev_gather[b], 0));
        c->gather_pending[b] = false;
    }
    float* pm = c->d_pmag[b];
    c->inten_live = false;
    const bool prof = c->prof_on && (size_t)(2 * c->prof_n + 1) < c->prof_ev.size();
    if (prof) HIPCHK(c, hipEventRecord(c->prof_ev[2 * c->prof_n], c->stream));
    if (c->hetero) { if (c->marched) olx_launch_hmarch(c, pm); else olx_launch_hetero(c, pm); }
    else if (c->use_mfma) {
        if (!c->use_lattice) olx_launch_mfma(c, pm);
        else if (c->use_coset) {
            auto go = [&](const LatticePart& q) { if (c->use_toep) olx_launch_toep(c, q, pm); else if (c->use_cosetp) olx_launch_cosetp(c, q, pm); else olx_launch_coset(c, q, pm); };
            if (c->fp8corr && c->cp_nfar < c->cp_nblocks) {
                if (c->cp_nfar) go(lattice_part(c, false));
                go(lattice_part(c, true));
            } else go(lattice_part(c, false));
        }
        else olx_launch_lattice(c, pm);
    }
    else if (c->mx * c->my * c->nf > 1) {
        if (!olx_launch_shared(c, pm)) return fail(c, OLX_ESTATE, "olx_field_launch: no kernel for variant %s", c->variant.c_str());
    } else if (c->modifier()) olx_launch_accum_dir(c, pm);
    else olx_launch_accum(c, pm);
    HIPCHK(c, hipGetLastError());
    if (prof) { HIPCHK(c, hipEventRecord(c->prof_ev[2 * c->prof_n + 1], c->stream)); c->prof_n++; }
    c->cur = b;
    return OLX_OK;
}

int olx_profile_begin(olx_ctx* c, int max_launches) {
    if (!c) return OLX_EINVAL;
    if (max_launches < 1 || max_launches > (1 << 20)) return fail(c, OLX_EINVAL, "olx_profile_begin: bad max_launches");
    HIPCHK(c, hipSetDevice(c->device));
    for (auto e : c->prof_ev) hipEventDestroy(e);
    c->prof_ev.assign(2 * (size_t)max_launches, nullptr);
    for (auto& e : c->prof_ev) HIPCHK(c, hipEventCreate(&e));
    c->prof_n = 0; c->prof_on = true;
    return OLX_OK;
}

int olx_profile_end(olx_ctx* c, float* ms_each, int capacity, int* n_recorded) {
    if (!c) return OLX_EINVAL;
    if (!ms_each || !n_recorded || capacity < 0) return fail(c, OLX_EINVAL, "olx_profile_end: null output");
    HIPCHK(c, hipSetDevice(c->device));
    HIPCHK(c, hipStreamSynchronize(c->stream));
    const int n = std::min(c->prof_n, capacity);
    for (int i = 0; i < n; ++i) HIPCHK(c, hipEventElapsedTime(&ms_each[i], c->prof_ev[2 * i], c->prof_ev[2 * i + 1]));
    *n_recorded = n;
    for (auto e : c->prof_ev) hipEventDestroy(e);
    c->prof_ev.clear(); c->prof_n = 0; c->prof_on = false;
    return OLX_OK;
}

}

struct FetchLane {
    static constexpr size_t CAPACITY = (size_t)8 << 20;
    hipStream_t stream = nullptr;
    void* buf[2] = {nullptr, nullptr};
    hipEvent_t ev[2] = {nullptr, nullptr};
    bool ok = false;
    void release() {
        for (int i = 0; i < 2; ++i) {
            if (ev[i]) hipEventDestroy(ev[i]);
            if (buf[i]) hipHostFree(buf[i]);
            ev[i] = nullptr; buf[i] = nullptr;
        }
        if (stream) hipStreamDestroy(stream);
        stream = nullptr; ok = false;
    }
    bool init() {
        if (ok) return true;
        release();
        bool good = hipStreamCreateWithFlags(&stream, hipStreamNonBlocking) == hipSuccess;
        for (int i = 0; good && i < 2; ++i)
            good = hipHostMalloc(&buf[i], CAPACITY, hipHostMallocDefault) == hipSuccess &&
                   hipEventCreateWithFlags(&ev[i], hipEventDisableTiming) == hipSuccess;
        if (!good) { (void)hipGetLastError(); release(); return false; }
        return ok = true;
    }
};
static constexpr int FETCH_MAX_THREADS = 32;
static FetchLane* ctx_fetch_lanes(olx_ctx* c) {
    if (!c->fetch_lanes) c->fetch_lanes = new FetchLane[FETCH_MAX_THREADS];
    return c->fetch_lanes;
}
static void free_fetch_lanes(olx_ctx* c) {
    if (!c->fetch_lanes) return;
    for (int t = 0; t < FETCH_MAX_THREADS; ++t) c->fetch_lanes[t].release();
    delete[] c->fetch_lanes;
    c->fetch_lanes = nullptr;
}

static hipError_t fetch_lane_run(int device, FetchLane& L, char* dst, const char* src, size_t lo, size_t hi, size_t chunk) {
    hipError_t e = hipSetDevice(device);
    if (e != hipSuccess) return e;
    const size_t n = (hi - lo + chunk - 1) / chunk;
    auto issue = [&](size_t i) {
        const size_t off = lo + i * chunk, cnt = std::min(chunk, hi - off);
        hipError_t r = hipMemcpyAsync(L.buf[i & 1], src + off, cnt, hipMemcpyDeviceToHost, L.stream);
        return r != hipSuccess ? r : hipEventRecord(L.ev[i & 1], L.stream);
    };
    if (n) { e = issue(0); if (e != hipSuccess) return e; }
    for (size_t i = 0; i < n; ++i) {
        if (i + 1 < n) { e = issue(i + 1); if (e != hipSuccess) return e; }
        e = hipEventSynchronize(L.ev[i & 1]);
        if (e != hipSuccess) return e;
        const size_t off = lo + i * chunk, cnt = std::min(chunk, hi - off);
        memcpy(dst + off, L.buf[i & 1], cnt);
    }
    return hipSuccess;
}

static int fetch_to_host(olx_ctx* c, void* dst, const void* src, size_t bytes) {
    const char* mode_env = getenv("OLX_FETCH_MODE");
    const int mode = !mode_env ? 2 : !strcmp(mode_env, "pageable") ? 0 : !strcmp(mode_env, "register") ? 1 : 2;
    if (mode == 1 && bytes >= ((size_t)1 << 20)) {
        if (hipHostRegister(dst, bytes, hipHostRegisterDefault) == hipSuccess) {
            hipError_t e = hipMemcpyAsync(dst, src, bytes, hipMemcpyDeviceToHost, c->stream);
            if (e == hipSuccess) e = hipStreamSynchronize(c->stream);
            hipHostUnregister(dst);
            if (e != hipSuccess) return fail(c, OLX_EHIP, "fetch (registered): %s", hipGetErrorString(e));
            return OLX_OK;
        }
        (void)hipGetLastError();
    }
    if (mode == 2 && bytes >= ((size_t)8 << 20)) {
        int nthr = 8;
        if (const char* t = getenv("OLX_FETCH_THREADS")) nthr = atoi(t);
        const int hw = (int)std::thread::hardware_concurrency();
        nthr = std::max(1, std::min({nthr, FETCH_MAX_THREADS, hw > 0 ? hw : 1, (int)(bytes >> 21)}));
        size_t chunk = std::min(FetchLane::CAPACITY, std::max((size_t)2 << 20, (bytes / nthr / 4 + 4095) & ~(size_t)4095));
        if (const char* t = getenv("OLX_FETCH_CHUNK_KB"))
            chunk = std::min(FetchLane::CAPACITY, std::max((size_t)64, (size_t)atol(t)) << 10);
        FetchLane* lanes = ctx_fetch_lanes(c);
        bool ready = true;
        for (int t = 0; t < nthr; ++t) ready = ready && lanes[t].init();
        if (ready) {
            const size_t per = ((bytes / nthr) + 4095) & ~(size_t)4095;
            std::vector<hipError_t> rc(nthr, hipSuccess);
            std::vector<std::thread> th;
            for (int t = 0; t < nthr; ++t) {
                const size_t lo = std::min(per * t, bytes), hi = t == nthr - 1 ? bytes : std::min(per * (t + 1), bytes);
                th.emplace_back([&, t, lo, hi] { rc[t] = fetch_lane_run(c->device, lanes[t], (char*)dst, (const char*)src, lo, hi, chunk); });
            }
            for (auto& t : th) t.join();
            for (int t = 0; t < nthr; ++t)
                if (rc[t] != hipSuccess) return fail(c, OLX_EHIP, "fetch (staged, worker %d): %s", t, hipGetErrorString(rc[t]));
            return OLX_OK;
        }
        (void)hipGetLastError();
    }
    HIPCHK(c, hipMemcpyAsync(dst, src, bytes, hipMemcpyDeviceToHost, c->stream));
    HIPCHK(c, hipStreamSynchronize(c->stream));
// ... 1742 lines not shown
```

openlifu-python_amd/csrc/olx_ctx.h:

```cpp
#pragma once
#include "../../include/olx.h"

#include <hip/hip_runtime.h>

#include <algorithm>
#include <cstdarg>
#include <cstdio>
#include <string>
#include <vector>

#include "olx_params.h"
#include "olx_plan.h"

using namespace olx;

typedef struct { char internal[OLX_UNIQUE_ID_BYTES]; } olx_nccl_id;
typedef void* olx_nccl_comm;
struct RcclApi {
    void* handle = nullptr;
    int (*GetUniqueId)(olx_nccl_id*) = nullptr;
    int (*CommInitRank)(olx_nccl_comm*, int, olx_nccl_id, int) = nullptr;
    int (*CommDestroy)(olx_nccl_comm) = nullptr;
    int (*AllGather)(const void*, void*, size_t, int , olx_nccl_comm, hipStream_t) = nullptr;
    int (*AllReduce)(const void*, void*, size_t, int , int , olx_nccl_comm, hipStream_t) = nullptr;
    int (*ReduceScatter)(const void*, void*, size_t , int , int , olx_nccl_comm, hipStream_t) = nullptr;
    const char* (*GetErrorString)(int) = nullptr;
    int (*CommCount)(olx_nccl_comm, int*) = nullptr;
};
static constexpr int kNcclFloat32 = 7;
static constexpr int kNcclSum = 0, kNcclMax = 2;

struct olx_ctx;

template <class T> class DevBuf {
    T* p = nullptr;
    size_t cap = 0;
public:
    DevBuf() = default;
    DevBuf(const DevBuf&) = delete;
    DevBuf& operator=(const DevBuf&) = delete;
    ~DevBuf() { release(); }
    int reserve(olx_ctx* c, size_t n);
    void release() { if (p) hipFree(p); p = nullptr; cap = 0; }
    size_t capacity() const { return cap; }
    operator T*() const { return p; }
};

struct FetchLane;
struct P2PState;

struct olx_ctx {
    int device = 0;
    FetchLane* fetch_lanes = nullptr;
    bool near = false;
    bool tab_split = false;
    int n_cu = 0;
    hipStream_t stream = nullptr;
    std::string err;
    int n_el = 0;
    DevBuf<double> d_pos, d_nrm, d_area;
    std::vector<double> h_pos;
    std::vector<double> h_area, h_delays, h_apod;
    std::vector<double> h_foci; unsigned long long foci_version = ~0ull;
    std::vector<double> h_xaxis, h_size, h_nrm; DevBuf<float> d_tab2; bool directivity = false; double absorb_np_m = 0; bool modifier() const { return directivity || absorb_np_m > 0; }
    bool dir_lattice = false;
    bool allow_shared = true;
    int n_foci = 0;
    DevBuf<double> d_delays, d_apod, d_foci, d_M;
    unsigned long long steer_version = 0, packed_version = ~0ull, configured_version = ~0ull;
    bool planned = false;
    double plan_absorb = 0;
    std::string plan_env;
    bool uploaded = false;
    olx_grid grid{};
    olx_slab slab{};
    int plan_foci = 0;
    double freq = 0, c = 0, rho = 0, p0_pa = 0;
    unsigned flags = 0;
    FieldParams fp{};
    bool flat = false, clamp = false;
    bool use_mfma = false; int nt = 1; MfmaParams mp{}; DevBuf<float4> d_coords; DevBuf<uint4> d_bfrag; DevBuf<int> d_colinfo;
    int* d_targets = nullptr;
    double min_dist = 0, mfma_wscale = 0; int force_kind = 0;
    int mx = 1, my = 1, dx = 1, dy = 1, nf = 1; std::vector<int> h_px, h_py; DevBuf<int> d_perm; SharedParams sp{};
    DevBuf<float> d_tab;
    typedef olxplan::Lattice Lattice;
    Lattice lat;
    bool use_lattice = false; int lat_mt = 8; LatParams lp{}; DevBuf<int> d_slot;
    std::vector<double> nf_s2;
    int fp8_kcut = 0;
    unsigned cp_nfar = 0;
    size_t bfrag_half = 0, afrag_half = 0;
    bool use_coset = false; bool fp8corr = false; CosetParams cp{}; DevBuf<int> d_jobs;
    DevBuf<CosetBlock> d_cpblocks; unsigned cp_nblocks = 0;
    int up_blocks_key[16] = {0};
    std::vector<CosetBlock> up_blocks; std::vector<int> up_jobs, up_slot;
    std::vector<int> up_perm, up_colinfo;
    bool use_cosetp = false;
    bool use_toep = false; int toep_nsa = 0, toep_saw = 16; unsigned toep_ksmask = 0; int toep_nm = 1;       int toep_targets[4] = {-1, -1, -1, -1};
    DevBuf<int> d_cell; DevBuf<uint4> d_afrag;
    static constexpr int NBUF = 2;
    DevBuf<float> d_pmag[NBUF];
    DevBuf<float> d_inten, d_cplx, d_agg_p, d_agg_i;
    bool derive_i = false;
    bool inten_live = false;
    DevBuf<float> d_ifetch;
    DevBuf<float> d_scale;
    DevBuf<double> d_peakA; DevBuf<unsigned> d_peak;
    DevBuf<float> d_wint;
    DevBuf<unsigned char> d_an; void* h_an = nullptr; size_t h_an_bytes = 0;
    bool an_pending = false; int an_F = 0, an_npts = 0; size_t an_out_pk = 0, an_out_ita = 0, an_out_bd = 0, an_out_mom = 0;
    bool hetero = false; HeteroParams hp{}; DevBuf<float4> d_med; DevBuf<int> d_plane_k, d_plane_of_k;
    DevBuf<float> d_inv2z; DevBuf<int> d_kfirst, d_klast;
    int planes_per_layer = 1;
    DevBuf<float4> d_med_layer; DevBuf<int> d_layer_lo, d_layer_hi;
    int medium_model = 0;
    bool march_one = false;
    DevBuf<float2> d_Utex;
    bool marched = false; DevBuf<float2> d_U[2]; std::vector<int> h_plane_k;
    DevBuf<float> d_sig;
    int nbuf = 1; int cur = 0;
    std::string variant;
    std::vector<hipEvent_t> prof_ev; int prof_n = 0; bool prof_on = false;
    double pulse_cycles = 0, pulse_dt = 0; int pulse_nt = 0;
    double pulse_plan_dt = 0;
    bool pulsed = false;
    bool pmax_live = false;
    bool agg_pmax_valid = false;
    PulseParams pulse{};
    DevBuf<float> d_pmax, d_agg_pmax;
    DevBuf<double4> d_ptab; DevBuf<float> d_pw;
    bool pii_live = false;
    int pii_foci = 0;
    long long pii_vox = 0;
    DevBuf<float> d_pii;
    bool pii_w_valid = false, pii_max_valid = false;
    DevBuf<float> d_pii_w, d_pii_max;
    DevBuf<float> d_pii_gw;
    DevBuf<double> d_pii_A;
    DevBuf<unsigned> d_pii_peak;
    DevBuf<long long> d_ptrace_vox; DevBuf<float> d_ptrace;
    bool th_planned = false, th_uniform = false; ThermalParams th{};
    double th_rate = 0;
    DevBuf<float> d_th_T[2]; int th_cur = 0; DevBuf<float> d_th_max, d_th_cem;
    DevBuf<float4> d_th_coef; DevBuf<float> d_th_irc, d_th_sfac; DevBuf<unsigned> d_th_rate;
    int th_steps = 0, th_max_focus = -1; std::vector<int> th_row; DevBuf<int> d_th_sf; DevBuf<float> d_th_tau;
    int th_npts = 0; DevBuf<long long> d_th_pts; DevBuf<float> d_th_trace;
    int th_src_foci = 0; bool th_src_resident = false; DevBuf<float> d_th_I;
    bool th_src_pii = false;
    int th_next = -1;
    DevBuf<float> d_sm_p; DevBuf<int> d_sm_n;
    DevBuf<double> d_sm_tabd; DevBuf<float> d_sm_tabf;
    DevBuf<double> d_sm_ap;
    bool sm_valid = false; SteerParams sm{}; int sm_kind = 0; bool sm_dir = false;
    DevBuf<float> d_smm_p; DevBuf<int> d_smm_n;
    DevBuf<float4> d_smm_med;
    DevBuf<int> d_smm_plane_k, d_smm_plane_of_k;
    DevBuf<float> d_smm_tabm;
    bool sm_medium = false; SteerMedParams smm{}; int smm_comp = 0; bool smm_phase = false;
    bool bm_set = false; BfMedParams bm{};
    DevBuf<double> d_bm_sig;
    DevBuf<double> d_bm_zp;
    DevBuf<int> d_bm_pk;
    std::vector<int> h_bm_pk;
    bool ba_set = false; BfMedParams ba{};
    DevBuf<double> d_ba_att;
    DevBuf<double> d_ba_zp;
    DevBuf<int> d_ba_pk;
    std::vector<int> h_ba_pk;
    DevBuf<double> d_ba_h;
    bool bc_valid = false; int bc_planes = 0;
    DevBuf<double> d_bc_zp;
    DevBuf<int2> d_bc_walk;
    P2PState* p2p = nullptr;
    bool comm_active() const { return comm != nullptr || p2p != nullptr; }
    RcclApi rccl; olx_nccl_comm comm = nullptr; int nranks = 1, rank = 0;
    hipStream_t comm_stream = nullptr; hipEvent_t ev_field[NBUF] = {nullptr, nullptr};
    hipEvent_t ev_gather[NBUF] = {nullptr, nullptr}; bool gather_pending[NBUF] = {false, false};
    DevBuf<float> d_gather;
    hipEvent_t ev_agg = nullptr, ev_red = nullptr; bool reduce_pending = false;
    int agg_local = -1, agg_total = 0;
    std::string rccl_path;
    bool bf_valid = false; double bf_c = 0, bf_scale = 1, bf_p0 = 0, bf_p1 = 0; int bf_kind = 0;
};

bool olx_p2p_requested();
bool olx_p2p_is_id(const void* id_bytes);
int olx_p2p_unique_id(olx_ctx* c, void* id_bytes);
int olx_p2p_init(olx_ctx* c, const void* id_bytes, int nranks, int rank);
int olx_p2p_destroy(olx_ctx* c);
int olx_p2p_attached(olx_ctx* c);
int olx_p2p_export(olx_ctx* c, void* blob_out);
int olx_p2p_import(olx_ctx* c, const void* blobs);
int olx_p2p_allgather(olx_ctx* c);
int olx_p2p_before_overwrite(olx_ctx* c, int b);
int olx_p2p_drain(olx_ctx* c);
int olx_p2p_aggregate(olx_ctx* c, bool scatter, bool with_i);
int olx_p2p_aggregate_before_overwrite(olx_ctx* c);

static inline int fail(olx_ctx* c, int code, const char* fmt, ...) {
    char buf[512];
    va_list ap; va_start(ap, fmt); vsnprintf(buf, sizeof buf, fmt, ap); va_end(ap);
    if (c) c->err = buf;
    return code;
}
#define HIPCHK(c, call)                                                                  \
    do {                                                                                 \
        hipError_t e_ = (call);                                                          \
        if (e_ != hipSuccess)                                                            \
            return fail((c), e_ == hipErrorOutOfMemory ? OLX_ENOMEM : OLX_EHIP, "%s: %s", #call, \
                        hipGetErrorString(e_));                                          \
    } while (0)

template <class T> int DevBuf<T>::reserve(olx_ctx* c, size_t n) {
    if (cap >= n && p) return OLX_OK;
    release();
    n = std::max(n, (size_t)1);
    HIPCHK(c, hipMalloc((void**)&p, sizeof(T) * n));
    cap = n;
    return OLX_OK;
}

static inline int reserve_aggregate(olx_ctx* c, bool with_p, bool with_i) {
    const size_t n = c->d_pmag[0].capacity();
    int rc = with_p ? c->d_agg_p.reserve(c, n) : OLX_OK;
    if (!rc && with_i) rc = c->d_agg_i.reserve(c, n);
    return rc;
}

static inline void pii_regrid(olx_ctx* c, long long vox) {
    c->pii_live = false; c->pii_w_valid = false; c->pii_max_valid = false;
    if (c->pii_vox != vox) { c->d_pii.release(); c->d_pii_w.release(); c->d_pii_max.release(); }
    c->pii_vox = vox;
}

struct DevScratch {
    void* p = nullptr;
    ~DevScratch() { if (p) hipFree(p); }
    template <class T> T* at(size_t byte_off) const { return reinterpret_cast<T*>(static_cast<unsigned char*>(p) + byte_off); }
};
```

openlifu-python_amd/csrc/olx_params.h:

```cpp
#pragma once
#ifdef __HIPCC__
#include <hip/hip_runtime.h>
#endif
#include <stdint.h>

namespace olx {

constexpr int BF_THREADS = 256;
constexpr int SH_HEAD = 8;
constexpr int TAB_STRIDE = 8;
constexpr int FIELD_THREADS = 256;

struct FieldParams {
    int nx, ny, nz;
    int n_el;
    int x_begin;
    float hx, hy, hz;
    float dmin2;
    float inten_scale;
    float flat_ez;
    float flat_kz, flat_fz;
    float absorb_l2;
    long long vox;
    unsigned flags;
};

struct SharedParams {
    int nx, ny, nz, n_el;
    int x_begin, n_foci;
    float hx, hy, hz;
    float dmin2, inten_scale, flat_ez;
    float flat_kz, flat_fz;
    long long vox;
    unsigned flags;
};

constexpr int MFMA_COLS = 8;
constexpr int MFMA_MAX_NT = 4;
constexpr int MFMA_ELEMS_LDS = 256;

struct MfmaParams {
    int nx, ny, nz, n_el_pad;
    int x_begin, n_tiles;
    float hx, hy, hz;
    float dmin2, flat_ez, g_scale;
    float flat_kz, flat_fz;
    float out_scale;
    float inten_scale;
    long long vox;
    unsigned flags;
};

struct LatParams {
    int nx, ny, nz;
    int x_lo, y_lo;
    int x_begin;
    int mx, my;
    int tiles_x, tiles_y;
    int kgroups;
    int nsa, nsb;
    int nsbp;
    int ux0, uy0;
    float fx0, fy0;
    float hx_hi, hx_lo, hy_hi, hy_lo, hz;
    float dmin2, flat_ez, g_scale, out_scale, inten_scale;
    long long vox;
    unsigned flags;
};

constexpr int LAT_ELEMS_LDS = 128;
constexpr int LAT_TW = 10;
constexpr int LAT_PSZ = 116;
constexpr int LAT_THREADS = 512;

struct CosetParams {
    int nx, ny, nz;
    int x_lo, y_lo, x_begin;
    int mx, my;
    int nsx, nsy;
    int xs;
    int kblocks;
    int nsa, nsb;
    int nsbp;
    int ux0, uy0;
    float fx0, fy0, hx_hi, hx_lo, hy_hi, hy_lo, hz;
    float dmin2, flat_ez, g_scale, out_scale, inten_scale;
    float dir_wx, dir_wy;
    float absorb_l2;
    long long vox;
    unsigned flags;
    int n_foci;
#ifdef OLX_DEV_PINS
    int cp_noreuse;
#endif
};

struct CosetBlock {
    int ibase, jbase;
    int k0;
    int npos;
    int KY;
    int ky_magic;
    int KX;
    int pad_;
};

constexpr int COS_NW = 8;
constexpr int COS_P = 2;
constexpr int COS_ZB = COS_NW * COS_P;
constexpr int COS_KYW = 11;
constexpr int COS_JOBS = 64;
constexpr int cos_kxw(int nt) { return nt >= 4 ? 2 : (nt >= 2 ? 3 : 6); }
constexpr bool cos_fp8(int nt) { return nt <= 2; }
constexpr float COS_F8_LO = 32.0f, COS_F8_HI = 1.0f / 64.0f;

constexpr int HET_TAB_HEAD = 12;

struct HeteroParams {
    int n_planes;
    int n_layers;
    int n_foci;
    float u0, v0;
    float inv_hx, inv_hy;
    int nxg, nyg;
    int xg_begin;
    float kappa;
};

struct PulseParams {
    int n_el, n_foci, n_t;
    int ny, nz;
    double ox, oy, oz, hx, hy, hz;
    double dmin;
    double inv_cdt;
    double tdt;
    double f0dt;
    float dmin_f, inv_cdt_f;
    float absorb;
    float rot_c, rot_s;
    float inten_scale;
    float pii_scale;
    long long vox;
};

struct ThermalParams {
    int nx, ny, nz;
    long long vox;
    float ihx2, ihy2, ihz2;
    float rho0, cp0, kappa0, alpha0;
    float perf;
    float gx, gy, gz;
    float irc0, sfac0;
};
struct ThermalStep {
    float dt;
    float dt_min;
    float tb43;
    int npts, n_foci;
};

struct BfMedParams {
    double ox, oy, oz, hx, hy, hz;
    double dmin;
    double ztol;
    double c;
    int nx, ny, nz, n_planes;
};

constexpr int STEER_TD = 8;
constexpr int STEER_TF = 16;
struct SteerParams {
    int n_el;
    int nx, ny, nz;
    long long vox;
    double ox, oy, oz, hx, hy, hz;
    double lim2;
    float dmin2;
    float value;
    float pw_scale, pw_off;
    float absorb_l2;
};

constexpr int STEER_TM = 4;
struct SteerMedParams {
    SteerParams S;
    double inv_hx, inv_hy;
    int n_planes;
    int spreading;
    float hz_w;
    float abs_value;
};

struct PeakParams {
    int nx, ny, nz;
    double ox, oy, oz, hx, hy, hz;
    double ia0, ia1, ia2;
    double radius; int op; int use_zmin; double zmin;
    long long vox;
    long long vol_stride;
};

}
```

openlifu-python_amd/csrc/olx_plan.cpp:

```cpp
#include "olx_plan.h"

#include "k_toep.hip.h"

#include <algorithm>
#include <climits>
#include <cmath>
#include <cstdlib>

namespace olxplan {

using namespace olx;

void build_slot_map(Lattice& L, int nsbp) {
    L.nsbp = nsbp; L.n_pad = L.nsa * nsbp * 64;
    L.slot_elem.assign((size_t)L.nsa * nsbp * 64, -1);
    for (int sa = 0; sa < L.nsa; ++sa)
        for (int sbb = 0; sbb < L.nsb; ++sbb)
            for (int ks = 0; ks < 4; ++ks)
                for (int bb = 0; bb < 4; ++bb)
                    for (int aa = 0; aa < 4; ++aa) {
                        const int a = 8 * sa + 4 * (ks & 1) + aa, b = 8 * sbb + 4 * (ks >> 1) + bb;
                        if (a < L.ax && b < L.ay)
                            L.slot_elem[((size_t)(sa * nsbp + sbb) * 4 + ks) * 16 + 4 * bb + aa] = L.cell[(size_t)a * L.ay + b];
                    }
}

void detect_lattice(Lattice& L, bool flat, int n, const double* pos, const double spacing[3], const double lo[3], const double hi[3], double dmin) {
    L = Lattice();
    if (!flat || n < 16 || n > 16384) return;
    const double* X = pos;
    const double* Y = X + n;
    const double tol = 1e-10;
    auto axis = [&](const double* v, std::vector<double>& u) {
        u.assign(v, v + n);
        std::sort(u.begin(), u.end());
        size_t m = 0;
        for (size_t q = 0; q < u.size(); ++q)
            if (m == 0 || u[q] - u[m - 1] > tol) u[m++] = u[q];
        u.resize(m);
    };
    std::vector<double> xs, ys;
    axis(X, xs); axis(Y, ys);
    const int ax = (int)xs.size(), ay = (int)ys.size();
    if (ax < 2 || ay < 2 || (long long)ax * ay != n) return;
    const double px = (xs.back() - xs.front()) / (ax - 1), py = (ys.back() - ys.front()) / (ay - 1);
    for (int a = 0; a < ax; ++a) if (std::fabs(xs[a] - (xs[0] + a * px)) > tol) return;
    for (int b = 0; b < ay; ++b) if (std::fabs(ys[b] - (ys[0] + b * py)) > tol) return;
    const double rx = px / spacing[0], ry = py / spacing[1];
    const int mx = (int)std::llround(rx), my = (int)std::llround(ry);
    if (mx < 1 || my < 1 || std::fabs(rx - mx) > 1e-9 * mx || std::fabs(ry - my) > 1e-9 * my) return;
    const int nsa = (ax + 7) / 8, nsb = (ay + 7) / 8;
    if ((long long)nsa * nsb * 64 > 2LL * n) return;
    std::vector<int> cell((size_t)ax * ay, -1);
    for (int e = 0; e < n; ++e) {
        const int a = (int)std::llround((X[e] - xs[0]) / px), b = (int)std::llround((Y[e] - ys[0]) / py);
        if (a < 0 || a >= ax || b < 0 || b >= ay || cell[(size_t)a * ay + b] >= 0) return;
        cell[(size_t)a * ay + b] = e;
    }
    L.ax = ax; L.ay = ay; L.nsa = nsa; L.nsb = nsb;
    L.cell.swap(cell);
    build_slot_map(L, nsb);
    const int nsbp = (nsb + 1) & ~1;
    const double ez = pos[2 * (size_t)n];
    double min_d2 = 1e300; bool clamp = false;
    const double guard = 2.0 * dmin;
    for (int a = 0; a < std::max(8 * nsa, 16 * ((ax + 15) / 16)); ++a)
        for (int b = 0; b < 8 * nsbp; ++b) {
            const double p[3] = {xs[0] + a * px, ys[0] + b * py, ez};
            double d2 = 0;
            for (int k = 0; k < 3; ++k) {
                const double d = p[k] < lo[k] ? lo[k] - p[k] : (p[k] > hi[k] ? p[k] - hi[k] : 0.0);
                d2 += d * d;
            }
            min_d2 = std::min(min_d2, d2);
            if (d2 < guard * guard) clamp = true;
        }
    L.mx = mx; L.my = my;
    L.x0 = xs[0]; L.y0 = ys[0]; L.px = px; L.py = py; L.min_d2 = min_d2; L.clamp = clamp;
    L.ok = true;
}

long long coset_tiles16(int wx, int wy, int mx, int my, int nt) {
    const int kxw = cos_kxw(nt);
    const int nsx = ((wx + 2 * mx - 1) / (2 * mx) + kxw - 1) / kxw, nsy = ((wy + my - 1) / my + COS_KYW - 1) / COS_KYW;
    long long t16 = 0;
    for (int rx = 0; rx < 2 * mx; ++rx)
        for (int ry = 0; ry < my; ++ry) {
            const int kxa = rx < wx ? (wx - 1 - rx) / (2 * mx) + 1 : 0, kya = ry < wy ? (wy - 1 - ry) / my + 1 : 0;
            for (int sx = 0; sx < nsx; ++sx)
                for (int sy = 0; sy < nsy; ++sy) {
                    const int KX = (sx + 1) * kxa / nsx - sx * kxa / nsx, KY = (sy + 1) * kya / nsy - sy * kya / nsy;
                    t16 += (COS_P * KX * KY + 15) / 16;
                }
        }
    return t16;
}

std::vector<int> mirror_perms(int n, int n_img, bool fold_x, bool fold_y, const int* px, const int* py, int rows) {
    std::vector<int> perm((size_t)rows * n);
    for (int m = 0; m < rows; ++m)
        for (int e = 0; e < n; ++e) {
            int o = e;
            const bool fx = fold_x && (m & 1), fy = fold_y && (fold_x ? (m >> 1) : (m & 1));
            if (m < n_img && fx) o = px[o];
            if (m < n_img && fy) o = py[o];
            perm[(size_t)m * n + e] = o;
        }
    return perm;
}

bool same_vector(const Steering& S, int f1, int m1, int f2, int m2) {
    const int n = S.n;
    for (int e = 0; e < n; ++e) {
        const size_t a = (size_t)f1 * n + S.perm[(size_t)m1 * n + e], b = (size_t)f2 * n + S.perm[(size_t)m2 * n + e];
        double dph = (S.delays[a] - S.delays[b]) * S.freq;
        dph -= std::nearbyint(dph);
        const double wa = S.apod[a] * S.area[a % n], wb = S.apod[b] * S.area[b % n];
        if (std::fabs(wa - wb) > 1e-12 * std::max(std::fabs(wa), std::fabs(wb))) return false;
        if (wa != 0.0 && std::fabs(dph) > 1e-9) return false;
    }
    return true;
}

Tiles pack_columns(const Steering& S, int maxc) {
    Tiles tl(1);
    for (int f = 0; f < S.F; ++f)
        for (int m = 0; m < S.n_img; ++m) {
            Col* hit = nullptr;
            for (size_t t = 0; t < tl.size() && !hit; ++t)
                for (size_t q = 0; q < tl[t].size() && !hit; ++q)
                    if (tl[t][q].ntgt < 4 && same_vector(S, tl[t][q].f, tl[t][q].m, f, m)) hit = &tl[t][q];
            if (!hit) {
                if ((int)tl.back().size() >= maxc) tl.emplace_back();
                tl.back().push_back(Col{f, m, 0, {-1, -1, -1, -1}});
                hit = &tl.back().back();
            }
            hit->tgt[hit->ntgt++] = f * 4 + m;
        }
    return tl;
}

void balance_store_targets(Tiles& tiles, int max_cols) {
    for (auto& t : tiles)
        for (size_t o = 0; o < t.size() && (int)t.size() < max_cols; ++o)
            if (t[o].ntgt > 2) {
                Col extra{t[o].f, t[o].m, 0, {-1, -1, -1, -1}};
                while (t[o].ntgt > 2) { extra.tgt[extra.ntgt++] = t[o].tgt[--t[o].ntgt]; t[o].tgt[t[o].ntgt] = -1; }
                t.push_back(extra);
            }
}

void coset_partition(CosetParams& Q, int kxw, int zb, int kyw) {
    const int px = Q.xs * Q.mx;
    const int kx_max = (Q.nx - Q.x_lo + px - 1) / px, ky_max = (Q.ny - Q.y_lo + Q.my - 1) / Q.my;
    Q.nsx = (kx_max + kxw - 1) / kxw; Q.nsy = (ky_max + kyw - 1) / kyw;
    Q.kblocks = (Q.nz + zb - 1) / zb;
}

bool build_coset_blocks(const CosetParams& Q, int zb, unsigned grp, int max_pos,
                        std::vector<CosetBlock>& blk, std::string& msg) {
    const int px = Q.xs * Q.mx;
    const unsigned nblk = (unsigned)(px * Q.my * Q.nsx * Q.nsy * Q.kblocks);
    blk.assign(nblk, CosetBlock{});
    const int wx = Q.nx - Q.x_lo, wy = Q.ny - Q.y_lo;
    for (unsigned id = 0; id < nblk; ++id) {
        unsigned b = id;
        int kblock, ry_lo = 0;
        unsigned gy = 1;
        if (grp > (unsigned)Q.kblocks && grp % (unsigned)Q.kblocks == 0 && (unsigned)Q.my % (grp / (unsigned)Q.kblocks) == 0 && nblk % (8 * grp) == 0) {
            gy = grp / (unsigned)Q.kblocks;
            const unsigned xcd = b % 8, sft = b / 8, inner = sft % grp;
            kblock = (int)(inner % (unsigned)Q.kblocks); ry_lo = (int)(inner / (unsigned)Q.kblocks);
            b = (sft / grp) * 8 + xcd;
        } else if (grp <= (unsigned)Q.kblocks && (Q.kblocks % grp) == 0 && nblk % (8 * grp) == 0) {
            const unsigned xcd = b % 8, sft = b / 8, kb_lo = sft % grp, u = (sft / grp) * 8 + xcd, part = (unsigned)Q.kblocks / grp;
            kblock = (int)(grp * (u % part) + kb_lo); b = u / part;
        } else { kblock = (int)(b % (unsigned)Q.kblocks); b /= (unsigned)Q.kblocks; }
        const int sy_part = (int)(b % (unsigned)Q.nsy); b /= (unsigned)Q.nsy;
        const int sx_part = (int)(b % (unsigned)Q.nsx); b /= (unsigned)Q.nsx;
        const unsigned myh = (unsigned)Q.my / gy;
        const int ry = (int)(b % myh) * (int)gy + ry_lo, rx = (int)(b / myh);
        const int kx_all = rx < wx ? (wx - 1 - rx) / px + 1 : 0, ky_all = ry < wy ? (wy - 1 - ry) / Q.my + 1 : 0;
        const int kx0 = sx_part * kx_all / Q.nsx, KX = (sx_part + 1) * kx_all / Q.nsx - kx0;
        const int ky0 = sy_part * ky_all / Q.nsy, KY = (sy_part + 1) * ky_all / Q.nsy - ky0;
        CosetBlock& B = blk[id];
        B.ibase = Q.x_lo + rx + px * kx0; B.jbase = Q.y_lo + ry + Q.my * ky0; B.k0 = kblock * zb;
        B.npos = (KX > 0 && KY > 0) ? KX * KY : 0; B.KY = KY > 0 ? KY : 1; B.ky_magic = 65536 / B.KY + 1; B.KX = KX > 0 ? KX : 0; B.pad_ = 0;
        if (max_pos > 0 && B.npos > max_pos) { msg = "a block part holds more than " + std::to_string(max_pos) + " positions"; return false; }
    }
    return true;
}

std::vector<int> build_store_jobs(const Tiles& tiles, int max_nt, int cols_per_nt, int jobs_per_tile, bool want_p, bool want_i) {
    const int ntiles = (int)tiles.size();
    std::vector<int> jobs((size_t)ntiles * max_nt * (jobs_per_tile + 1), -1);
    for (int t = 0; t < ntiles; ++t)
        for (int nt = 0; nt < max_nt; ++nt) {
            int* jb = &jobs[((size_t)t * max_nt + nt) * (jobs_per_tile + 1)];
            int cnt = 0;
            for (int c16 = 0; c16 < 16; ++c16) {
                const bool wantp = (c16 & 1) ? want_i : want_p;
                const size_t o = (size_t)nt * cols_per_nt + (c16 >> 1);
                if (!wantp || o >= tiles[t].size()) continue;
                for (int q = 0; q < 4; ++q) {
                    const int code = tiles[t][o].tgt[q];
                    if (code >= 0) jb[cnt++] = c16 | ((code & 3) << 4) | ((code >> 2) << 6);
                }
            }
            int lg = 0;
            while ((1 << lg) < cnt) ++lg;
            jb[jobs_per_tile] = lg;
        }
    return jobs;
}

bool infer_foci(bool flat, int n, int F, const double* pos, const double* delays, double c, double grid_z_mid, std::vector<double>& foci) {
    if (!flat || n < 4 || !delays) return false;
    const double* X = pos; const double* Y = X + n; const double* Z = Y + n;
    foci.assign(3 * (size_t)F, 0.0);
    for (int f = 0; f < F; ++f) {
        const double* tau = delays + (size_t)f * n;
        double A[3][4] = {{0}};
        const double s0 = c * tau[0], q0 = X[0] * X[0] + Y[0] * Y[0];
        for (int e = 1; e < n; ++e) {
            const double se = c * tau[e];
            const double row[3] = {-2.0 * (X[e] - X[0]), -2.0 * (Y[e] - Y[0]), 2.0 * (se - s0)};
            const double rhs = (se * se - s0 * s0) - (X[e] * X[e] + Y[e] * Y[e] - q0);
            for (int i = 0; i < 3; ++i) {
                for (int j = 0; j < 3; ++j) A[i][j] += row[i] * row[j];
                A[i][3] += row[i] * rhs;
            }
        }
        for (int i = 0; i < 3; ++i) {
            int piv = i;
            for (int r = i + 1; r < 3; ++r) if (std::fabs(A[r][i]) > std::fabs(A[piv][i])) piv = r;
            if (!(std::fabs(A[piv][i]) > 1e-300)) return false;
            if (piv != i) for (int j = 0; j < 4; ++j) std::swap(A[i][j], A[piv][j]);
            for (int r = 0; r < 3; ++r) {
                if (r == i) continue;
                const double m = A[r][i] / A[i][i];
                for (int j = i; j < 4; ++j) A[r][j] -= m * A[i][j];
            }
        }
        const double x = A[0][3] / A[0][0], y = A[1][3] / A[1][1], S = A[2][3] / A[2][2];
        const double dz2 = (S - s0) * (S - s0) - (x - X[0]) * (x - X[0]) - (y - Y[0]) * (y - Y[0]);
        if (!(dz2 > 0) || !std::isfinite(dz2)) return false;
        const double side = grid_z_mid >= Z[0] ? 1.0 : -1.0;
        const double z = Z[0] + side * std::sqrt(dz2);
        for (int e = 0; e < n; ++e) {
            const double d = std::sqrt((x - X[e]) * (x - X[e]) + (y - Y[e]) * (y - Y[e]) + (z - Z[e]) * (z - Z[e]));
            if (!(std::fabs(d - (S - c * tau[e])) <= 1e-6)) return false;
        }
        foci[3 * (size_t)f] = x; foci[3 * (size_t)f + 1] = y; foci[3 * (size_t)f + 2] = z;
    }
    return true;
}

double nearfield_s2(int n, const double* pos, const double origin[3], const double spacing[3], const int begin[3], const int count[3], double dclamp) {
    if (n <= 0) return 0.0;
    const double* P[3] = {pos, pos + n, pos + 2 * (size_t)n};
    const double dc2 = dclamp * dclamp;
    const int stride = n <= 1024 ? 1 : (n + 1023) / 1024;
    int centre = 0;
    {
        double m[3] = {0, 0, 0}, best = 1e300;
        for (int a = 0; a < 3; ++a) { for (int e = 0; e < n; ++e) m[a] += P[a][e]; m[a] /= n; }
        for (int e = 0; e < n; ++e) {
            double d2 = 0;
            for (int a = 0; a < 3; ++a) d2 += (P[a][e] - m[a]) * (P[a][e] - m[a]);
            if (d2 < best) { best = d2; centre = e; }
        }
    }
    std::vector<int> cand;
    for (int e = 0; e < n; e += stride) cand.push_back(e);
    cand.push_back(centre);
    double s2max = 0.0;
    for (const int e0 : cand) {
        double v[3];
        for (int a = 0; a < 3; ++a) {
            long long i = std::llround((P[a][e0] - origin[a]) / spacing[a]);
            i = std::max<long long>(begin[a], std::min<long long>(i, (long long)begin[a] + count[a] - 1));
            v[a] = origin[a] + (double)i * spacing[a];
        }
        double s2 = 0.0;
        for (int e = 0; e < n; ++e) {
            const double dx = v[0] - P[0][e], dy = v[1] - P[1][e], dz = v[2] - P[2][e];
            s2 += 1.0 / std::max(dx * dx + dy * dy + dz * dz, dc2);
        }
        s2max = std::max(s2max, s2);
    }
    return s2max;
}

int fp8_first_plane(int n, const double* pos, const double* area, const double* apod, int F, const double* foci, const double origin[3],
                    const double spacing[3], const int gn[3], int x_begin, int x_count, const Lattice& L, std::vector<double>& nf_s2) {
    bool ok = true;
    double need = 0;
    for (int f = 0; ok && f < F; ++f) {
        for (int a = 0; a < 3; ++a) {
            const int b0 = a == 0 ? x_begin : 0, cnt = a == 0 ? x_count : gn[a];
            const double lo = origin[a] + (b0 - 0.5) * spacing[a];
            const double hi = origin[a] + (b0 + cnt - 0.5) * spacing[a];
            if (!(foci[3 * (size_t)f + a] >= lo && foci[3 * (size_t)f + a] <= hi)) ok = false;
        }
        double sw1 = 0, sw2 = 0, wmx = 0, peak = 0;
        const double* fo = &foci[3 * (size_t)f];
        for (int e = 0; e < n; ++e) {
            const double w = std::fabs(apod[(size_t)f * n + e] * area[e]);
            sw1 += w; sw2 += w * w; wmx = std::max(wmx, w);
            const double ddx = fo[0] - pos[e], ddy = fo[1] - pos[(size_t)n + e], ddz = fo[2] - pos[2 * (size_t)n + e];
            peak += w / std::sqrt(std::max(ddx * ddx + ddy * ddy + ddz * ddz, 1e-30));
        }
        if (!(sw2 > 0 && sw1 * sw1 / sw2 >= 255.5) || !(peak > 0)) ok = false;
        else need = std::max(need, FP8_ERR_K * wmx / (FP8_ERR_BOUND * peak));
    }
    if (!ok) return -1;
    {
        int planes = 0;
        for (int a = 0; a < 2; ++a) {
            const double ctr = (a == 0 ? L.x0 + 0.5 * (L.ax - 1) * L.px : L.y0 + 0.5 * (L.ay - 1) * L.py);
            const double idx = (ctr - origin[a]) / spacing[a];
            const int b0 = a == 0 ? x_begin : 0, cnt = a == 0 ? x_count : gn[a];
            if (std::fabs(idx - std::round(idx)) <= 1e-6 && idx >= b0 - 0.5 && idx <= b0 + cnt - 0.5) ++planes;
        }
        need *= 1.0 + 0.25 * planes;
    }
    const int nzb = (gn[2] + COS_ZB - 1) / COS_ZB;
    if ((int)nf_s2.size() != nzb) nf_s2.assign(nzb, -1.0);
    for (int q = 0; q < nzb; ++q) {
        if (nf_s2[q] < 0) {
            const int b0[3] = {x_begin, 0, q * COS_ZB}, cnt[3] = {x_count, gn[1], gn[2] - q * COS_ZB};
            nf_s2[q] = nearfield_s2(n, pos, origin, spacing, b0, cnt, 0.5 * std::min({spacing[0], spacing[1], spacing[2]}));
        }
        if (need * std::sqrt(nf_s2[q]) <= 1.0) return q * COS_ZB;
    }
    return -1;
}

bool fp8_split_pays(int x_count, int ny, int nz, int F, int cut) {
    return !((double)x_count * ny * (nz - cut) * F < 8.0e6 || 4 * cut > nz);
}

ToepPlan toep_plan(int ax, int mx, int my, int xs, int wx, int wy, int nz, bool dir_lattice, int saw_pin, int nm_pin) {
    ToepPlan T{};
    T.saw = std::min(ax, saw_pin ? saw_pin : 24);
    T.nm = T.saw + 15 <= 32 ? 2 : 1;
    T.kyw = COS_KYW;
    const int zb = COS_ZB;
    const int kxa_max = wx > 0 ? (wx - 1) / (xs * mx) + 1 : 0, kya_max = wy > 0 ? (wy - 1) / my + 1 : 0;
    auto parts = [](int k, int w) { return std::max(1, (k + w - 1) / w); };
    if (T.nm == 2) {
        if ((kxa_max + parts(kxa_max, 16) - 1) / parts(kxa_max, 16) <= 8) T.nm = 1;
    } else if (!dir_lattice) {
        auto slots = [&](int nm, int kyw_, int nky) {
            const int px_ = parts(kxa_max, 8 * nm), py_ = parts(kya_max, kyw_);
            const int ky_part = (kya_max + py_ - 1) / py_;
            return (long long)px_ * 8 * nm * py_ * ((ky_part + nky - 1) / nky) * nky;
        };
        const long long nblk3 = (long long)xs * mx * my * parts(kxa_max, 24) * parts(kya_max, ToepShape<3>::KYW) * ((nz + zb - 1) / zb);
        const bool want3 = nm_pin ? nm_pin == 3 : (kxa_max > 8 && nblk3 >= 256 && 20 * slots(3, ToepShape<3>::KYW, ToepShape<3>::NKY) <= 21 * slots(1, ToepShape<1>::KYW, ToepShape<1>::NKY));
        if (want3) { T.nm = 3; T.kyw = ToepShape<3>::KYW; }
    }
    T.nsa = (ax + T.saw - 1) / T.saw;
    if (T.nsa > 16) return T;
    for (int sa = 0; sa < T.nsa; ++sa) {
        const int wdt = std::min(T.saw, ax - sa * T.saw);
        const int lo_c = T.saw - wdt, hi_c = T.saw - 1 + xs * (8 - 1);
        unsigned m = 0;
        if (lo_c <= 15) m |= 1u;
        if (hi_c >= 16) m |= 2u;
        T.ks_mask |= m << (2 * sa);
        T.ksteps_total += (int)(m & 1u) + (int)(m >> 1);
        T.e4_units += (T.nm == 3 && m == 2u) ? 1 : 2;
    }
    return T;
}

}
```

openlifu-python_amd/csrc/olx_plan.h:

```cpp
#pragma once
#include <string>
#include <vector>

#include "olx_params.h"

namespace olxplan {

using olx::CosetBlock;
using olx::CosetParams;

struct Lattice {
    bool ok = false;
    int ax = 0, ay = 0, nsa = 0, nsb = 0, mx = 1, my = 1, n_pad = 0;
    double x0 = 0, y0 = 0, px = 0, py = 0;
    double min_d2 = 0; bool clamp = false;
    std::vector<int> slot_elem;
    std::vector<int> cell;
    int nsbp = 0;
};

void build_slot_map(Lattice& L, int nsbp);

void detect_lattice(Lattice& L, bool flat, int n, const double* pos, const double spacing[3], const double lo[3], const double hi[3], double dmin);

long long coset_tiles16(int wx, int wy, int mx, int my, int nt);

std::vector<int> mirror_perms(int n, int n_img, bool fold_x, bool fold_y, const int* px, const int* py, int rows);

struct Col { int f, m, ntgt; int tgt[4]; };
typedef std::vector<std::vector<Col>> Tiles;

struct Steering {
    int n = 0, F = 0, n_img = 1;
    const int* perm = nullptr;
    const double* delays = nullptr;
    const double* apod = nullptr;
    const double* area = nullptr;
    double freq = 0;
};
bool same_vector(const Steering& S, int f1, int m1, int f2, int m2);
Tiles pack_columns(const Steering& S, int maxc);
void balance_store_targets(Tiles& tiles, int max_cols);

void coset_partition(CosetParams& Q, int kxw, int zb, int kyw = olx::COS_KYW);

bool build_coset_blocks(const CosetParams& Q, int zb, unsigned grp, int max_pos, std::vector<CosetBlock>& blk, std::string& msg);

std::vector<int> build_store_jobs(const Tiles& tiles, int max_nt, int cols_per_nt, int jobs_per_tile, bool want_p, bool want_i);

bool infer_foci(bool flat, int n, int F, const double* pos , const double* delays , double c, double grid_z_mid,
                std::vector<double>& foci);

constexpr double FP8_ERR_K = 3.75e-5;
constexpr double FP8_ERR_BOUND = 7.5e-6;
double nearfield_s2(int n, const double* pos, const double origin[3], const double spacing[3], const int begin[3], const int count[3], double dclamp);

int fp8_first_plane(int n, const double* pos, const double* area, const double* apod, int F, const double* foci, const double origin[3],
                    const double spacing[3], const int gn[3], int x_begin, int x_count, const Lattice& L, std::vector<double>& nf_s2);
bool fp8_split_pays(int x_count, int ny, int nz, int F, int cut);

struct ToepPlan {
    int saw, nsa;
    int nm, kyw;
    unsigned ks_mask;
    int ksteps_total;
    int e4_units;
};
ToepPlan toep_plan(int ax, int mx, int my, int xs, int wx, int wy, int nz, bool dir_lattice, int saw_pin = 0, int nm_pin = 0);

}
```

Measured before the change: 111.1 million.

## Chain x-parts of a coset into one block and share overlapping Toeplitz columns

```diff
diff --git a/openlifu-python_amd/csrc/k_coset2.hip b/openlifu-python_amd/csrc/k_coset2.hip
--- a/openlifu-python_amd/csrc/k_coset2.hip
+++ b/openlifu-python_amd/csrc/k_coset2.hip
@@ -21,11 +21,12 @@
 #endif
 
 template <int MX, int MY, bool CLAMP, bool FP8, bool DIR = false, bool BOTH = true ,
-          bool PONLY = false >
+          bool PONLY = false ,
+          bool CHAIN = false >
 __global__ __launch_bounds__(COS_NW * 64, 4) void field_cosetp_k(
     const uint4* __restrict__ bfrag, float* __restrict__ pmag, float* __restrict__ inten,
     const int* __restrict__ targets ,
-    const CosetBlock* __restrict__ blocks , const CosetParams P) {
+    const void* __restrict__ blocks , const CosetParams P) {
     constexpr int NT = 2, THREADS = COS_NW * 64, PAIR = 2;
     static_assert(!(BOTH && PONLY), "one output or both");
     constexpr int TROWS = CP_TROWS, ROW0 = CP_ROW0, PSZ = CP_PSZ, MT = CP_MT;
@@ -44,12 +45,54 @@
     OLX_CUTRACE(0, (unsigned long long)__builtin_amdgcn_s_getreg((31 << 11) | 4));
     OLX_CUTRACE(1, (unsigned long long)__builtin_amdgcn_s_getreg((31 << 11) | 20));
     const int item = blockIdx.x;
-    {
-    const CosetBlock BK = blocks[item];
-    const int npos = BK.npos, KY = BK.KY, ky_magic = BK.ky_magic;
-    if (npos <= 0) return;
-    const int ibase = BK.ibase, jbase = BK.jbase;
-    const int k0 = BK.k0;
+    int KY, ky_magic, jbase, k0, pk0 = 0, pk1 = 0, pk2 = 0, pk3 = 0, npos1 = 0, ibase1 = 0;
+    if constexpr (CHAIN) {
+        const CosetChain BK = static_cast<const CosetChain*>(blocks)[item];
+        KY = BK.KY; ky_magic = BK.ky_magic; jbase = BK.jbase; k0 = BK.k0;
+        static_assert(COS_CHAIN_PARTS == 4, "the part selects below");
+        auto pack = [](int ib, int kx, int np) { return (int)(((unsigned)ib << 8) | ((unsigned)kx << 6) | (unsigned)np); };
+        pk0 = pack(BK.ibase[0], BK.KX[0], BK.npos[0]); pk1 = pack(BK.ibase[1], BK.KX[1], BK.npos[1]);
+        pk2 = pack(BK.ibase[2], BK.KX[2], BK.npos[2]); pk3 = pack(BK.ibase[3], BK.KX[3], BK.npos[3]);
+        if (((pk0 | pk1 | pk2 | pk3) & 63) == 0) return;
+    } else {
+        const CosetBlock BK = static_cast<const CosetBlock*>(blocks)[item];
+        KY = BK.KY; ky_magic = BK.ky_magic; jbase = BK.jbase; k0 = BK.k0; npos1 = BK.npos; ibase1 = BK.ibase;
+        if (npos1 <= 0) return;
+    }
+    const int nsbp = P.nsbp;
+    const int n_sb = P.nsa * nsbp;
+    bool reuse_ok = nsbp == PAIR;
+    bool share_ok = CHAIN && nsbp == PAIR && P.nsa <= 2;
+#ifdef OLX_DEV_PINS
+    reuse_ok = reuse_ok && P.cp_noreuse == 0;
+    share_ok = share_ok && P.cp_noreuse == 0 && P.cp_noshare == 0;
+#endif
+    constexpr int CHUNK_U4 = PAIR * 4 * NT * B_KS_U4, PRE = CHUNK_U4 / THREADS;
+    static_assert(CHUNK_U4 % THREADS == 0, "chunk must split evenly over the block");
+    uint4 pre[PRE];
+    const uint4* const bsrc = bfrag + (size_t)tile * n_sb * (4 * NT * B_KS_U4);
+#pragma unroll
+    for (int q = 0; q < PRE; ++q) {
+        const int idx = tid + q * THREADS;
+        pre[q] = idx < n_sb * 4 * NT * B_KS_U4 ? bsrc[idx] : make_uint4(0, 0, 0, 0);
+    }
+    bool chained = false;
+    constexpr int NPARTS = CHAIN ? COS_CHAIN_PARTS : 1;
+#ifdef OLX_EXP_CP_UNROLL
+#pragma unroll
+#else
+#pragma nounroll
+#endif
+    for (int part = NPARTS - 1; part >= 0; --part) {
+    int npos = npos1, ibase = ibase1, KXp = 0;
+    bool more = false;
+    if constexpr (CHAIN) {
+        const int pk = part == 3 ? pk3 : part == 2 ? pk2 : part == 1 ? pk1 : pk0;
+        npos = pk & 63;
+        if (npos == 0) continue;
+        ibase = (int)((unsigned)pk >> 8); KXp = (pk >> 6) & 3;
+        more = (((part >= 1 ? pk0 : 0) | (part >= 2 ? pk1 : 0) | (part >= 3 ? pk2 : 0)) & 63) != 0;
+    }
     const int ntile = __builtin_amdgcn_readfirstlane((npos - wave + COS_NW - 1) / COS_NW);
     const int lane_off = p16 * PSZ - g * CP_TW;
     int toff[MT];
@@ -64,26 +107,12 @@
     for (int t = 0; t < MT; ++t)
 #pragma unroll
         for (int nt = 0; nt < NT; ++nt) acc[t][nt] = floatx4_t{0.f, 0.f, 0.f, 0.f};
-    const int nsbp = P.nsbp;
-    const int n_sb = P.nsa * nsbp;
-    bool reuse_ok = nsbp == PAIR;
-#ifdef OLX_DEV_PINS
-    reuse_ok = reuse_ok && P.cp_noreuse == 0;
-#endif
-    constexpr int CHUNK_U4 = PAIR * 4 * NT * B_KS_U4, PRE = CHUNK_U4 / THREADS;
-    static_assert(CHUNK_U4 % THREADS == 0, "chunk must split evenly over the block");
-    uint4 pre[PRE];
-    const uint4* const bsrc = bfrag + (size_t)tile * n_sb * (4 * NT * B_KS_U4);
-#pragma unroll
-    for (int q = 0; q < PRE; ++q) {
-        const int idx = tid + q * THREADS;
-        pre[q] = idx < n_sb * 4 * NT * B_KS_U4 ? bsrc[idx] : make_uint4(0, 0, 0, 0);
-    }
     OLX_STAMP(0);
     for (int sb0 = 0; sb0 < n_sb; sb0 += PAIR) {
         const int sa = sb0 / nsbp, sbb0 = sb0 - sa * nsbp;
         if (sb0 > 0) __syncthreads();
         const bool reuse = sb0 > 0 && reuse_ok;
+        const bool share = CHAIN && sb0 == 0 && chained && share_ok;
         if (sb0 == 0) OLX_STAMP(1);
         if (sb0 == 2) OLX_STAMP(7);
         if constexpr (FP8) __builtin_amdgcn_s_setprio(1);
@@ -167,7 +196,40 @@
                     entry(fmaf(dy, dy, dx2), dzl, dx, dy, (wave * COS_P + wl) * PSZ + (TROWS - 1) * CP_TW + (CP_UW - 1 - ui), wl < COS_P);
                 }
             };
-            if (reuse) {
+            if (share) {
+                static_assert(COS_P * TROWS <= 64 && CP_UW == 12 && CP_TW % 2 == 0 && PSZ % 2 == 0, "one lane per (plane, row); aligned 8-byte moves");
+                const int d = 2 * KXp;
+                const int m_src = P.nsa == 2 ? 0 : d, m_dst = P.nsa == 2 ? 8 - d : 0;
+                const int n8 = (CP_UW - m_src - m_dst) / 2;
+                const int zm = lane_o >= TROWS ? 1 : 0;
+                const int mo = (wave * COS_P + zm) * PSZ + (lane_o - zm * TROWS) * CP_TW;
+                if (lane_o < COS_P * TROWS && OLX_IN(mo, T_WORDS - (CP_UW - 1), 4)) {
+#pragma unroll
+                    for (int arr = 0; arr < 2; ++arr) {
+                        unsigned* const tb = (arr ? s_lo : s_hi) + mo;
+                        unsigned long long mv[CP_UW / 2 - 1];
+#pragma unroll
+                        for (int q = 0; q < CP_UW / 2 - 1; ++q) __builtin_memcpy(&mv[q], __builtin_assume_aligned(tb + m_src + 2 * min(q, n8 - 1), 8), 8);
+#pragma unroll
+                        for (int q = 0; q < CP_UW / 2 - 1; ++q) __builtin_memcpy(__builtin_assume_aligned(tb + m_dst + 2 * min(q, n8 - 1), 8), &mv[q], 8);
+                    }
+                }
+                __builtin_amdgcn_fence(__ATOMIC_RELEASE, "wavefront");
+                const int row = lane_o >> 1, col = lane_o & 1;
+                const bool last_row = KY + 14 >= TROWS - 1;
+                const bool row_ok = row < TROWS - 1 || (row == TROWS - 1 && last_row);
+                const float W = (float)(jbase + P.uy0 + P.my * (row - ROW0));
+                const float dy = fmaf(W, P.hy_hi, fmaf(W, P.hy_lo, P.fy0));
+                const int w_end = P.nsa == 2 ? 8 - d : CP_UW;
+                for (int w0 = (P.nsa == 2 ? 6 : CP_UW) - d; w0 < w_end; w0 += 2) {
+                    const int ui = CP_UW - 1 - (w0 + col);
+                    const float U = (float)(ibase + P.x_begin + P.ux0 + P.mx * (ui - 7));
+                    const float dx = fmaf(U, P.hx_hi, fmaf(U, P.hx_lo, P.fx0));
+                    const float r2 = fmaf(dy, dy, dx * dx);
+#pragma unroll
+                    for (int z = 0; z < COS_P; ++z) entry(r2, dz2[z], dx, dy, (wave * COS_P + z) * PSZ + row * CP_TW + w0 + col, row_ok);
+                }
+            } else if (reuse) {
                 static_assert(COS_P * TROWS <= 64 && CP_UW - CP_SHARED == 8 && CP_TW % 2 == 0 && PSZ % 2 == 0, "one lane per (plane, row); aligned 8-byte moves");
                 const int zm = lane_o >= TROWS ? 1 : 0;
                 const int mo = (wave * COS_P + zm) * PSZ + (lane_o - zm * TROWS) * CP_TW;
@@ -195,7 +257,8 @@
         __syncthreads();
         if (sb0 == 0) OLX_STAMP(3);
         {
-            const int nxt = (sb0 + PAIR) * 4 * NT * B_KS_U4, lim = n_sb * 4 * NT * B_KS_U4;
+            const int lim = n_sb * 4 * NT * B_KS_U4;
+            const int nxt = sb0 + PAIR < n_sb ? (sb0 + PAIR) * 4 * NT * B_KS_U4 : (more ? 0 : lim);
 #pragma unroll
             for (int q = 0; q < PRE; ++q) {
                 const int idx = nxt + tid + q * THREADS;
@@ -290,6 +353,7 @@
         if (sb0 == 0) OLX_STAMP(4);
     }
     OLX_STAMP(5);
+    chained = true;
     int lane_e = lane;
     asm volatile("" : "+v"(lane_e));
     const int c16 = lane_e >> 2;
@@ -368,12 +432,17 @@
     if (k0 + COS_ZB <= P.nz) readout(IntC<1>{}); else readout(IntC<0>{});
     }
     OLX_STAMP(6);
+    if (more) {
+        __builtin_amdgcn_fence(__ATOMIC_RELEASE, "workgroup", "local");
+        __builtin_amdgcn_s_barrier();
+        __builtin_amdgcn_fence(__ATOMIC_ACQUIRE, "workgroup", "local");
+    }
+    }
 #ifdef OLX_EXP_CUTRACE
     OLX_CUTRACE(3, __builtin_readcyclecounter());
     asm volatile("s_waitcnt vmcnt(0)" ::: "memory");
     OLX_CUTRACE(4, __builtin_readcyclecounter());
 #endif
-    }
 }
 
 }
@@ -401,10 +470,12 @@
     float* inten_exp = c->d_inten;
     const bool clamp = c->clamp || c->lat.clamp;
     dim3 grid(q.n_blocks, c->mp.n_tiles), blk(COS_NW * 64);
+    const void* const recs = q.blocks;
     const bool both = (Q.flags & 3u) == 3u, ponly = (Q.flags & 3u) == 1u;
-#define OLX_CP(CL, F8, DR) do { if (both) hipLaunchKernelGGL((field_cosetp_k<MX, MY, CL, F8, DR, true, false>), grid, blk, 0, c->stream, q.bfrag, pm, inten_exp, c->d_targets, q.blocks, Q); \
-                                else if (ponly) hipLaunchKernelGGL((field_cosetp_k<MX, MY, CL, F8, DR, false, true>), grid, blk, 0, c->stream, q.bfrag, pm, inten_exp, c->d_targets, q.blocks, Q); \
-                                else hipLaunchKernelGGL((field_cosetp_k<MX, MY, CL, F8, DR, false, false>), grid, blk, 0, c->stream, q.bfrag, pm, inten_exp, c->d_targets, q.blocks, Q); } while (0)
+#define OLX_CP3(CL, F8, DR, CH) do { if (both) hipLaunchKernelGGL((field_cosetp_k<MX, MY, CL, F8, DR, true, false, CH>), grid, blk, 0, c->stream, q.bfrag, pm, inten_exp, c->d_targets, recs, Q); \
+                                else if (ponly) hipLaunchKernelGGL((field_cosetp_k<MX, MY, CL, F8, DR, false, true, CH>), grid, blk, 0, c->stream, q.bfrag, pm, inten_exp, c->d_targets, recs, Q); \
+                                else hipLaunchKernelGGL((field_cosetp_k<MX, MY, CL, F8, DR, false, false, CH>), grid, blk, 0, c->stream, q.bfrag, pm, inten_exp, c->d_targets, recs, Q); } while (0)
+#define OLX_CP(CL, F8, DR) do { if (c->cp_chained) OLX_CP3(CL, F8, DR, true); else OLX_CP3(CL, F8, DR, false); } while (0)
     if (c->dir_lattice) {
         if (clamp) OLX_CP(true, false, true); else OLX_CP(false, false, true);
     } else if (q.fp8) {
@@ -413,6 +484,7 @@
         if (clamp) OLX_CP(true, false, false); else OLX_CP(false, false, false);
     }
 #undef OLX_CP
+#undef OLX_CP3
 }
 
 void olx_launch_cosetp(olx_ctx* c, const LatticePart& q, float* pm) {
diff --git a/openlifu-python_amd/csrc/olx.hip b/openlifu-python_amd/csrc/olx.hip
--- a/openlifu-python_amd/csrc/olx.hip
+++ b/openlifu-python_amd/csrc/olx.hip
@@ -710,7 +710,15 @@
                 Q.vox = L.vox; Q.flags = L.flags; Q.n_foci = F;
 #ifdef OLX_DEV_PINS
                 { const char* e = getenv("OLX_EXP_CP_NOREUSE"); Q.cp_noreuse = (e && atoi(e) != 0) ? 1 : 0; }
+                { const char* e = getenv("OLX_EXP_CP_NOSHARE"); Q.cp_noshare = (e && atoi(e) != 0) ? 1 : 0; }
 #endif
+                bool chained = c->use_cosetp && Q.nsx >= 2 && Q.nsx <= COS_CHAIN_PARTS && Q.nsbp == 2 && Q.nsa <= 2;
+#ifdef OLX_DEV_PINS
+                bool nochain_pin = false;
+                if (const char* e = getenv("OLX_EXP_CP_NOCHAIN")) nochain_pin = chained && atoi(e) != 0;
+                if (nochain_pin) chained = false;
+#endif
+                const int nsx_ids = chained ? 1 : Q.nsx;
                 Q.dir_wx = (c->dir_lattice && c->directivity) ? (float)(0.5 * c->h_size[0] / lambda) : 0.f;
                 Q.dir_wy = (c->dir_lattice && c->directivity) ? (float)(0.5 * c->h_size[1] / lambda) : 0.f;
                 Q.absorb_l2 = c->dir_lattice ? (float)(c->absorb_np_m * lambda * 1.4426950408889634) : 0.f;
@@ -721,7 +729,7 @@
                 }
                 {
                     auto pick_grp = [&](int kblocks) {
-                        const unsigned long long nb = (unsigned long long)Q.xs * Q.mx * Q.my * Q.nsx * Q.nsy * kblocks;
+                        const unsigned long long nb = (unsigned long long)Q.xs * Q.mx * Q.my * nsx_ids * Q.nsy * kblocks;
                         for (int g2 = std::min(kblocks, 32); g2 >= 2; --g2) if (kblocks % g2 == 0 && nb % (8ull * g2) == 0) return (unsigned)g2;
                         return 1u;
                     };
@@ -731,25 +739,37 @@
 #ifdef OLX_DEV_PINS
                     if (const char* e = getenv("OLX_EXP_KGRP")) { kgrp = (unsigned)std::max(1, atoi(e)); if (kb_near > 0) kgrp_near = kgrp; }
 #endif
-                    const int rec_key[16] = {Q.nx, Q.ny, Q.nz, Q.x_lo, Q.y_lo, Q.mx, Q.my, Q.nsx, Q.nsy, Q.kblocks, zb, (int)kgrp, c->use_cosetp ? 40 : 0, Q.xs, kcut, (int)kgrp_near};
+                    const int rec_key[17] = {Q.nx, Q.ny, Q.nz, Q.x_lo, Q.y_lo, Q.mx, Q.my, Q.nsx, Q.nsy, Q.kblocks, zb, (int)kgrp, c->use_cosetp ? 40 : 0, Q.xs, kcut, (int)kgrp_near, chained ? 1 : 0};
+                    static_assert(sizeof rec_key == sizeof c->up_blocks_key, "the context keeps the whole key");
+                    c->cp_chained = chained;
+                    c->cp_slots = chained ? 2u : 1u;
                     std::vector<CosetBlock> blk;
                     if (!c->up_blocks.empty() && memcmp(c->up_blocks_key, rec_key, sizeof rec_key) == 0) blk = c->up_blocks;
                     else {
                         std::string why;
-                        CosetParams Qf = Q; Qf.kblocks = kb_far;
-                        if (!olxplan::build_coset_blocks(Qf, zb, kgrp, c->use_cosetp ? 40 : 0, blk, why))
-                            return fail(c, OLX_ESTATE, "kernel 2g: %s", why.c_str());
-                        for (CosetBlock& b : blk) b.k0 += kcut;
+                        auto side = [&](int kb, unsigned grp, int kfirst, std::vector<CosetBlock>& out) -> bool {
+                            CosetParams Qs = Q; Qs.kblocks = kb;
+                            if (!chained) {
+                                if (!olxplan::build_coset_blocks(Qs, zb, grp, c->use_cosetp ? 40 : 0, out, why)) return false;
+                                for (CosetBlock& b : out) b.k0 += kfirst;
+                                return true;
+                            }
+                            std::vector<CosetChain> rec;
+                            if (!olxplan::build_coset_chains(Qs, zb, grp, 40, rec, why)) return false;
+                            for (CosetChain& r : rec) r.k0 += kfirst;
+                            out.resize(2 * rec.size());
+                            if (!rec.empty()) memcpy(out.data(), rec.data(), sizeof(CosetChain) * rec.size());
+                            return true;
+                        };
+                        if (!side(kb_far, kgrp, kcut, blk)) return fail(c, OLX_ESTATE, "kernel 2g: %s", why.c_str());
                         if (kb_near > 0) {
                             std::vector<CosetBlock> near;
-                            CosetParams Qn = Q; Qn.kblocks = kb_near;
-                            if (!olxplan::build_coset_blocks(Qn, zb, kgrp_near, c->use_cosetp ? 40 : 0, near, why))
-                                return fail(c, OLX_ESTATE, "kernel 2g: %s", why.c_str());
+                            if (!side(kb_near, kgrp_near, 0, near)) return fail(c, OLX_ESTATE, "kernel 2g: %s", why.c_str());
                             blk.insert(blk.end(), near.begin(), near.end());
                         }
                     }
-                    const unsigned nblk = (unsigned)blk.size();
-                    c->cp_nfar = nblk - (unsigned)((unsigned long long)Q.xs * Q.mx * Q.my * Q.nsx * Q.nsy * kb_near);
+                    const unsigned nblk = (unsigned)(blk.size() / c->cp_slots);
+                    c->cp_nfar = nblk - (unsigned)((unsigned long long)Q.xs * Q.mx * Q.my * nsx_ids * Q.nsy * kb_near);
                     { int rc = upload_if_changed(c, c->d_cpblocks, c->up_blocks, blk); if (rc) return rc; }
                     memcpy(c->up_blocks_key, rec_key, sizeof rec_key);
                     c->cp_nblocks = nblk;
@@ -796,13 +816,13 @@
                     n_mfma = (long long)((double)npos_all * Q.kblocks * A.nsa * A.nsb * 4 * c->nt * corr_units * ntiles);
                 }
 #ifdef OLX_DEV_PINS
-                const char* const noreuse_tag = (c->use_cosetp && Q.cp_noreuse) ? ",noreuse" : "";
+                const std::string pin_tag = std::string(nochain_pin ? ",nochain" : "") + ((c->use_cosetp && Q.cp_noshare) ? ",noshare" : "") + ((c->use_cosetp && Q.cp_noreuse) ? ",noreuse" : "");
 #else
-                const char* const noreuse_tag = "";
+                const std::string pin_tag;
 #endif
                 snprintf(nmbuf, sizeof nmbuf, "field_coset%s_k<nt%d,mx%d,my%d,flat,%s%s%s> %d columns for %d foci x %d images in %d tile(s); "
                          "%dx%d lattice, pitch %dx%d voxels, %lld MFMA/launch (%lld dense)", c->use_cosetp ? "p" : "", c->nt, c->mx, c->my, lat_clamp ? "clamp" : "noclamp",
-                         f8tag.c_str(), noreuse_tag, total_cols, F, n_img, ntiles, A.ax, A.ay, A.mx, A.my, n_mfma, n_dense);
+                         f8tag.c_str(), pin_tag.c_str(), total_cols, F, n_img, ntiles, A.ax, A.ay, A.mx, A.my, n_mfma, n_dense);
                 }
             } else {
                 const long long n_mfma = (long long)L.tiles_x * L.tiles_y * L.kgroups * A.nsa * A.nsb * 4 * c->lat_mt * c->nt * 3 * ntiles;
@@ -838,7 +858,7 @@
 }
 
 static LatticePart lattice_part(const olx_ctx* c, bool below) {
-    if (below) return {c->d_bfrag + c->bfrag_half, c->d_afrag + c->afrag_half, c->d_cpblocks + c->cp_nfar, c->cp_nblocks - c->cp_nfar, false};
+    if (below) return {c->d_bfrag + c->bfrag_half, c->d_afrag + c->afrag_half, c->d_cpblocks + (size_t)c->cp_nfar * c->cp_slots, c->cp_nblocks - c->cp_nfar, false};
     const bool split = c->fp8corr && c->cp_nfar < c->cp_nblocks;
     return {c->d_bfrag, c->d_afrag, c->d_cpblocks, split ? c->cp_nfar : c->cp_nblocks, c->fp8corr};
 }
@@ -980,7 +1000,7 @@
     HIPCHK(c, hipSetDevice(c->device));
     {
         std::string env;
-        for (const char* name : {"OLX_FIELD_VARIANT", "OLX_FP8_CORRECTION", "OLX_EXP_TOEP_SAW", "OLX_EXP_TOEP_NM", "OLX_EXP_KGRP", "OLX_INTENSITY_STORED", "OLX_EXP_CP_NOREUSE"}) { const char* e = getenv(name); env += e ? e : ""; env += '|'; }
+        for (const char* name : {"OLX_FIELD_VARIANT", "OLX_FP8_CORRECTION", "OLX_EXP_TOEP_SAW", "OLX_EXP_TOEP_NM", "OLX_EXP_KGRP", "OLX_INTENSITY_STORED", "OLX_EXP_CP_NOREUSE", "OLX_EXP_CP_NOSHARE", "OLX_EXP_CP_NOCHAIN"}) { const char* e = getenv(name); env += e ? e : ""; env += '|'; }
         const bool same = c->planned && !c->uploaded && !c->hetero && !c->pulsed && memcmp(&c->grid, g, sizeof *g) == 0 && c->slab.x_begin == s.x_begin &&
                           c->slab.x_count == s.x_count && c->plan_foci == n_foci && c->freq == freq && c->c == cs && c->rho == rho &&
                           c->p0_pa == p0_pa && c->flags == flags && c->plan_absorb == c->absorb_np_m && c->nbuf == (c->comm_active() ? olx_ctx::NBUF : 1) && c->plan_env == env;
diff --git a/openlifu-python_amd/csrc/olx_ctx.h b/openlifu-python_amd/csrc/olx_ctx.h
--- a/openlifu-python_amd/csrc/olx_ctx.h
+++ b/openlifu-python_amd/csrc/olx_ctx.h
@@ -93,7 +93,9 @@
     size_t bfrag_half = 0, afrag_half = 0;
     bool use_coset = false; bool fp8corr = false; CosetParams cp{}; DevBuf<int> d_jobs;
     DevBuf<CosetBlock> d_cpblocks; unsigned cp_nblocks = 0;
-    int up_blocks_key[16] = {0};
+    bool cp_chained = false;
+    unsigned cp_slots = 1;
+    int up_blocks_key[17] = {0};
     std::vector<CosetBlock> up_blocks; std::vector<int> up_jobs, up_slot;
     std::vector<int> up_perm, up_colinfo;
     bool use_cosetp = false;
diff --git a/openlifu-python_amd/csrc/olx_params.h b/openlifu-python_amd/csrc/olx_params.h
--- a/openlifu-python_amd/csrc/olx_params.h
+++ b/openlifu-python_amd/csrc/olx_params.h
@@ -92,6 +92,7 @@
     int n_foci;
 #ifdef OLX_DEV_PINS
     int cp_noreuse;
+    int cp_noshare;
 #endif
 };
 
@@ -104,6 +105,16 @@
     int KX;
     int pad_;
 };
+
+constexpr int COS_CHAIN_PARTS = 4;
+struct CosetChain {
+    int jbase, k0;
+    int KY, ky_magic;
+    int ibase[COS_CHAIN_PARTS];
+    int KX[COS_CHAIN_PARTS];
+    int npos[COS_CHAIN_PARTS];
+};
+static_assert(sizeof(CosetChain) == 2 * sizeof(CosetBlock), "two 32-byte scalar loads; two slots of the record buffer");
 
 constexpr int COS_NW = 8;
 constexpr int COS_P = 2;
diff --git a/openlifu-python_amd/csrc/olx_plan.cpp b/openlifu-python_amd/csrc/olx_plan.cpp
--- a/openlifu-python_amd/csrc/olx_plan.cpp
+++ b/openlifu-python_amd/csrc/olx_plan.cpp
@@ -157,6 +157,31 @@
     Q.kblocks = (Q.nz + zb - 1) / zb;
 }
 
+namespace {
+struct BlockId { int kblock, sy_part, sx_part, rx, ry; };
+BlockId decode_block_id(const CosetParams& Q, int nsx_ids, unsigned grp, unsigned nblk, unsigned id) {
+    unsigned b = id;
+    int kblock, ry_lo = 0;
+    unsigned gy = 1;
+    if (grp > (unsigned)Q.kblocks && grp % (unsigned)Q.kblocks == 0 && (unsigned)Q.my % (grp / (unsigned)Q.kblocks) == 0 && nblk % (8 * grp) == 0) {
+        gy = grp / (unsigned)Q.kblocks;
+        const unsigned xcd = b % 8, sft = b / 8, inner = sft % grp;
+        kblock = (int)(inner % (unsigned)Q.kblocks); ry_lo = (int)(inner / (unsigned)Q.kblocks);
+        b = (sft / grp) * 8 + xcd;
+    } else if (grp <= (unsigned)Q.kblocks && (Q.kblocks % grp) == 0 && nblk % (8 * grp) == 0) {
+        const unsigned xcd = b % 8, sft = b / 8, kb_lo = sft % grp, u = (sft / grp) * 8 + xcd, part = (unsigned)Q.kblocks / grp;
+        kblock = (int)(grp * (u % part) + kb_lo); b = u / part;
+    } else { kblock = (int)(b % (unsigned)Q.kblocks); b /= (unsigned)Q.kblocks; }
+    BlockId d;
+    d.kblock = kblock;
+    d.sy_part = (int)(b % (unsigned)Q.nsy); b /= (unsigned)Q.nsy;
+    d.sx_part = (int)(b % (unsigned)nsx_ids); b /= (unsigned)nsx_ids;
+    const unsigned myh = (unsigned)Q.my / gy;
+    d.ry = (int)(b % myh) * (int)gy + ry_lo; d.rx = (int)(b / myh);
+    return d;
+}
+}
+
 bool build_coset_blocks(const CosetParams& Q, int zb, unsigned grp, int max_pos,
                         std::vector<CosetBlock>& blk, std::string& msg) {
     const int px = Q.xs * Q.mx;
@@ -164,29 +189,37 @@
     blk.assign(nblk, CosetBlock{});
     const int wx = Q.nx - Q.x_lo, wy = Q.ny - Q.y_lo;
     for (unsigned id = 0; id < nblk; ++id) {
-        unsigned b = id;
-        int kblock, ry_lo = 0;
-        unsigned gy = 1;
-        if (grp > (unsigned)Q.kblocks && grp % (unsigned)Q.kblocks == 0 && (unsigned)Q.my % (grp / (unsigned)Q.kblocks) == 0 && nblk % (8 * grp) == 0) {
-            gy = grp / (unsigned)Q.kblocks;
-            const unsigned xcd = b % 8, sft = b / 8, inner = sft % grp;
-            kblock = (int)(inner % (unsigned)Q.kblocks); ry_lo = (int)(inner / (unsigned)Q.kblocks);
-            b = (sft / grp) * 8 + xcd;
-        } else if (grp <= (unsigned)Q.kblocks && (Q.kblocks % grp) == 0 && nblk % (8 * grp) == 0) {
-            const unsigned xcd = b % 8, sft = b / 8, kb_lo = sft % grp, u = (sft / grp) * 8 + xcd, part = (unsigned)Q.kblocks / grp;
-            kblock = (int)(grp * (u % part) + kb_lo); b = u / part;
-        } else { kblock = (int)(b % (unsigned)Q.kblocks); b /= (unsigned)Q.kblocks; }
-        const int sy_part = (int)(b % (unsigned)Q.nsy); b /= (unsigned)Q.nsy;
-        const int sx_part = (int)(b % (unsigned)Q.nsx); b /= (unsigned)Q.nsx;
-        const unsigned myh = (unsigned)Q.my / gy;
-        const int ry = (int)(b % myh) * (int)gy + ry_lo, rx = (int)(b / myh);
+        const BlockId d = decode_block_id(Q, Q.nsx, grp, nblk, id);
+        const int sx_part = d.sx_part, sy_part = d.sy_part, rx = d.rx, ry = d.ry;
         const int kx_all = rx < wx ? (wx - 1 - rx) / px + 1 : 0, ky_all = ry < wy ? (wy - 1 - ry) / Q.my + 1 : 0;
         const int kx0 = sx_part * kx_all / Q.nsx, KX = (sx_part + 1) * kx_all / Q.nsx - kx0;
         const int ky0 = sy_part * ky_all / Q.nsy, KY = (sy_part + 1) * ky_all / Q.nsy - ky0;
         CosetBlock& B = blk[id];
-        B.ibase = Q.x_lo + rx + px * kx0; B.jbase = Q.y_lo + ry + Q.my * ky0; B.k0 = kblock * zb;
+        B.ibase = Q.x_lo + rx + px * kx0; B.jbase = Q.y_lo + ry + Q.my * ky0; B.k0 = d.kblock * zb;
         B.npos = (KX > 0 && KY > 0) ? KX * KY : 0; B.KY = KY > 0 ? KY : 1; B.ky_magic = 65536 / B.KY + 1; B.KX = KX > 0 ? KX : 0; B.pad_ = 0;
         if (max_pos > 0 && B.npos > max_pos) { msg = "a block part holds more than " + std::to_string(max_pos) + " positions"; return false; }
+    }
+    return true;
+}
+
+bool build_coset_chains(const CosetParams& Q, int zb, unsigned grp, int max_pos,
+                        std::vector<CosetChain>& rec, std::string& msg) {
+    if (Q.nsx > COS_CHAIN_PARTS) { msg = "more than " + std::to_string(COS_CHAIN_PARTS) + " x parts per coset"; return false; }
+    const int px = Q.xs * Q.mx;
+    const unsigned nblk = (unsigned)(px * Q.my * Q.nsy * Q.kblocks);
+    rec.assign(nblk, CosetChain{});
+    const int wx = Q.nx - Q.x_lo, wy = Q.ny - Q.y_lo;
+    for (unsigned id = 0; id < nblk; ++id) {
+        const BlockId d = decode_block_id(Q, 1, grp, nblk, id);
+        const int kx_all = d.rx < wx ? (wx - 1 - d.rx) / px + 1 : 0, ky_all = d.ry < wy ? (wy - 1 - d.ry) / Q.my + 1 : 0;
+        const int ky0 = d.sy_part * ky_all / Q.nsy, KY = (d.sy_part + 1) * ky_all / Q.nsy - ky0;
+        CosetChain& R = rec[id];
+        R.jbase = Q.y_lo + d.ry + Q.my * ky0; R.k0 = d.kblock * zb; R.KY = KY > 0 ? KY : 1; R.ky_magic = 65536 / R.KY + 1;
+        for (int s = 0; s < Q.nsx; ++s) {
+            const int kx0 = s * kx_all / Q.nsx, KX = (s + 1) * kx_all / Q.nsx - kx0;
+            R.ibase[s] = Q.x_lo + d.rx + px * kx0; R.KX[s] = KX > 0 ? KX : 0; R.npos[s] = (KX > 0 && KY > 0) ? KX * KY : 0;
+            if (max_pos > 0 && R.npos[s] > max_pos) { msg = "a block part holds more than " + std::to_string(max_pos) + " positions"; return false; }
+        }
     }
     return true;
 }
diff --git a/openlifu-python_amd/csrc/olx_plan.h b/openlifu-python_amd/csrc/olx_plan.h
--- a/openlifu-python_amd/csrc/olx_plan.h
+++ b/openlifu-python_amd/csrc/olx_plan.h
@@ -7,6 +7,8 @@
 namespace olxplan {
 
 using olx::CosetBlock;
+using olx::CosetChain;
+using olx::COS_CHAIN_PARTS;
 using olx::CosetParams;
 
 struct Lattice {
@@ -46,6 +48,8 @@
 
 bool build_coset_blocks(const CosetParams& Q, int zb, unsigned grp, int max_pos, std::vector<CosetBlock>& blk, std::string& msg);
 
+bool build_coset_chains(const CosetParams& Q, int zb, unsigned grp, int max_pos, std::vector<CosetChain>& rec, std::string& msg);
+
 std::vector<int> build_store_jobs(const Tiles& tiles, int max_nt, int cols_per_nt, int jobs_per_tile, bool want_p, bool want_i);
 
 bool infer_foci(bool flat, int n, int F, const double* pos , const double* delays , double c, double grid_z_mid,
```

After: 112.0 million (median of 6 runs). About the same (+0.9%).
